# lyndonchan/wsss-analysis

Measured on AMD Instinct MI355X. Metric: images/sec CAM+CRF pseudo-labels, VOC2012 321x321, higher is better.
Workload: dtype f16x3; 1 GPU; resnet50 CAM + dense-CRF (M=21, 10 mean-field iters), 321x321, batch 32 images (=64 samples) per GPU, image-sharded; batch_images=32, num_classes=20, parallelism=image-sharded x1, no collective, steps_per_rank=239

## Files before the change

__graft_entry__.py:

```python
import os
import subprocess
import sys

ROOT = os.path.dirname(os.path.abspath(__file__))
PKG_DIR = os.path.join(ROOT, "wsss-analysis_amd")
CSRC = os.path.join(PKG_DIR, "csrc")
LIB_OUT = os.path.join(PKG_DIR, "wsscam", "libwsscam.so")
ORACLE_DIR = os.path.join(ROOT, "oracle")
ORACLE_OUT = os.path.join(ORACLE_DIR, "_build", "libdensecrf_ref.so")

HIP_SOURCES = ["api.hip", "conv_igemm.hip", "misc_kernels.hip", "net.hip", "cam_tail.hip", "crf.hip", "irn_kernels.hip", "rw.hip", "hsn.hip", "input.hip", "ir_label.hip", "stem_pool.hip", "cam_head.hip", "conv_f32.hip", "dsrg.hip", "cue_seeds.hip", "seg_eval.hip", "deeplab.hip", "seg_chain.hip", "seg_loss.hip", "pool.hip", "seg_grad.hip", "seg_sgd.hip", "seg_dropout.hip"]
EXTRA_FLAGS = {"crf.hip": ["-ffp-contract=off"], "input.hip": ["-ffp-contract=off"], "deeplab.hip": ["-ffp-contract=off"],
               "seg_chain.hip": ["-ffp-contract=off"],
               "seg_sgd.hip": ["-ffp-contract=off"],
               "seg_dropout.hip": ["-ffp-contract=off"]}


def _newer(target, deps):
    if not os.path.exists(target):
        return False
    t = os.path.getmtime(target)
    return all(os.path.getmtime(d) <= t for d in deps)


def _run(cmd):
    r = subprocess.run(cmd, stdout=subprocess.PIPE, stderr=subprocess.STDOUT, text=True)
    if r.returncode != 0:
        raise RuntimeError("command failed: %s\n%s" % (" ".join(cmd), r.stdout))
    return r.stdout


def build_lib(force=False, verbose=False):
    hipcc = os.environ.get("HIPCC", "/opt/rocm/bin/hipcc")
    objdir = os.path.join(PKG_DIR, "build")
    os.makedirs(objdir, exist_ok=True)
    os.makedirs(os.path.dirname(LIB_OUT), exist_ok=True)
    headers = [os.path.join(CSRC, "common.h"), os.path.join(CSRC, "bilerp.h"), os.path.join(CSRC, "tf_resize.h"),
               os.path.join(ROOT, "include", "wsscam.h")]
    if not force and _newer(LIB_OUT, [os.path.join(CSRC, src) for src in HIP_SOURCES] + headers):
        return LIB_OUT
    objs = []
    procs = []
    for src in HIP_SOURCES:
        sp = os.path.join(CSRC, src)
        op = os.path.join(objdir, src.replace(".hip", ".o"))
        objs.append(op)
        if not force and _newer(op, [sp] + headers):
            continue
        cmd = [hipcc, "--offload-arch=gfx950", "-O3", "-std=c++17", "-fPIC", "-Wall", "-c", sp, "-o", op] + EXTRA_FLAGS.get(src, [])
        if verbose:
            print(" ".join(cmd))
        procs.append((cmd, subprocess.Popen(cmd, stdout=subprocess.PIPE, stderr=subprocess.STDOUT, text=True)))
    for cmd, p in procs:
        out, _ = p.communicate()
        if p.returncode != 0:
            raise RuntimeError("hipcc failed: %s\n%s" % (" ".join(cmd), out))
        if verbose and out.strip():
            print(out)
    if force or procs or not _newer(LIB_OUT, objs):
        _run([hipcc, "--offload-arch=gfx950", "-shared", "-fPIC", "-o", LIB_OUT] + objs)
    return LIB_OUT


def build_oracle(force=False):
    src = os.path.join(ORACLE_DIR, "densecrf_ref.c")
    os.makedirs(os.path.dirname(ORACLE_OUT), exist_ok=True)
    if force or not _newer(ORACLE_OUT, [src]):
        _run(["gcc", "-O2", "-fPIC", "-shared", "-ffp-contract=off", "-o", ORACLE_OUT, src, "-lm"])
    return ORACLE_OUT


def build():
    build_lib()
    build_oracle()
    if PKG_DIR not in sys.path:
        sys.path.insert(0, PKG_DIR)
    import wsscam

    wsscam._lib.check_exports()


def smoke():
    if PKG_DIR not in sys.path:
        sys.path.insert(0, PKG_DIR)
    if ROOT not in sys.path:
        sys.path.insert(0, ROOT)
    from tests import smoke_impl

    smoke_impl.run()


if __name__ == "__main__":
    build_lib(force="--force" in sys.argv, verbose=True)
    build_oracle(force="--force" in sys.argv)
    print("built", LIB_OUT)
```

include/wsscam.h:

```cpp
#ifndef WSSCAM_H
#define WSSCAM_H

#include <stddef.h>
#include <stdint.h>

#ifdef __cplusplus
extern "C" {
#endif

#define WSC_VERSION 100

typedef enum wsc_status {
    WSC_OK = 0,
    WSC_ERR_INVALID = -1,
    WSC_ERR_NO_DEVICE = -2,
    WSC_ERR_HIP = -3,
    WSC_ERR_MISSING_KEY = -4,
    WSC_ERR_SHAPE = -5,
    WSC_ERR_NOMEM = -6,
    WSC_ERR_KEY_RANGE = -7,
    WSC_ERR_CAPACITY = -8,
    WSC_ERR_RANGE = -9
} wsc_status;

typedef enum wsc_arch {
    WSC_ARCH_RESNET50_CAM = 0,
    WSC_ARCH_VGG16_CAM = 1,
    WSC_ARCH_M7_CAM = 2,
    WSC_ARCH_RESNET50_IRN = 3,
    WSC_ARCH_VGG16_IRN = 4,
    WSC_ARCH_M7_IRN = 5,
    WSC_ARCH_DEEPLAB_LFOV = 6,
    WSC_ARCH_DEEPLAB_ASPP = 7
} wsc_arch;

typedef enum wsc_precision {
    WSC_PREC_BF16 = 0,
    WSC_PREC_BF16X3 = 1,
    WSC_PREC_F16 = 2,
    WSC_PREC_F16X3 = 3,
    WSC_PREC_F32 = 4
} wsc_precision;

typedef struct wsc_ctx wsc_ctx;
typedef struct wsc_net wsc_net;
typedef enum {
    WSC_OPT_CRF_GAUSS_ON_CHIP = 0,
    WSC_OPT_CRF_FUSED_BLUR = 1,
    WSC_OPT_CRF_BLUR_ON_CHIP = 2,
    WSC_OPT_CRF_RANK_BALLOT = 3,
    WSC_OPT_CRF_EMBED_FULL = 4,
    WSC_OPT_RW_TILED = 5,
    WSC_OPT_STEM_POOL_FUSED = 6,
    WSC_OPT_CONV_WINDOW = 7,
    WSC_OPT_CAM_HEAD_STREAM = 8,
    WSC_OPT_CRF_MSG_IN_UPDATE = 9,
    WSC_OPT_COUNT = 10
} wsc_option;

typedef struct wsc_crf wsc_crf;
typedef struct wsc_crf_v wsc_crf_v;

typedef struct wsc_tensor_desc {
    const char *name;
    const float *data;
    int32_t ndim;
    int64_t shape[4];
} wsc_tensor_desc;


int wsc_version(void);
const char *wsc_last_error(void);

int wsc_ctx_create(int device, void *stream, wsc_ctx **out);
void wsc_ctx_destroy(wsc_ctx *ctx);
int wsc_ctx_set_option(wsc_ctx *ctx, int option, int value);
int wsc_sync(wsc_ctx *ctx);
int wsc_ctx_range_status(wsc_ctx *ctx, int *flag_out, int clear);
int wsc_ctx_wait(wsc_ctx *ctx, wsc_ctx *other);
int wsc_ctx_mark(wsc_ctx *ctx, int slot);
int wsc_ctx_wait_mark(wsc_ctx *ctx, int slot);
int wsc_ctx_wait_for_mark(wsc_ctx *ctx, wsc_ctx *other, int slot);
int wsc_device_info(wsc_ctx *ctx, char *arch_name, size_t arch_name_len, int *num_cus);

int wsc_malloc(wsc_ctx *ctx, size_t bytes, void **dptr_out);
int wsc_free(wsc_ctx *ctx, void *dptr);
int wsc_memcpy_h2d(wsc_ctx *ctx, void *dst_dev, const void *src_host, size_t bytes);
int wsc_memcpy_d2h(wsc_ctx *ctx, void *dst_host, const void *src_dev, size_t bytes);
int wsc_memset(wsc_ctx *ctx, void *dst_dev, int value, size_t bytes);
int wsc_host_alloc(wsc_ctx *ctx, size_t bytes, void **host_out);
int wsc_host_free(wsc_ctx *ctx, void *host);
int wsc_host_write_segments(const char *path, int n, const void *const *ptrs, const size_t *sizes);
int wsc_memcpy_h2d_async(wsc_ctx *ctx, void *dst_dev, const void *src_pinned_host, size_t bytes);
int wsc_memcpy_d2h_async(wsc_ctx *ctx, void *dst_pinned_host, const void *src_dev, size_t bytes);

int wsc_timer_begin(wsc_ctx *ctx);
int wsc_timer_end(wsc_ctx *ctx, float *ms_out);

int wsc_profile_begin(wsc_ctx *ctx);
int wsc_profile_end(wsc_ctx *ctx, int max_classes, int32_t *calls_out, float *total_ms_out, double *work_out,
                    int *n_classes_out);
const char *wsc_profile_class_name(int cls);


int wsc_net_create(wsc_ctx *ctx, int arch, const wsc_tensor_desc *weights, int n_weights,
                   int num_classes, int precision, wsc_net **out);
void wsc_net_destroy(wsc_net *net);
int wsc_net_cam_size(const wsc_net *net, int S, int *h_out);
int wsc_net_feat_channels(const wsc_net *net, int *f_out);

int wsc_net_forward_cam(wsc_ctx *ctx, const wsc_net *net, const float *x_dev, int B, int S,
                        float *cam_dev, float *score_dev);
int wsc_net_cam_size_hw(const wsc_net *net, int H, int W, int *h_out, int *w_out);
int wsc_net_forward_cam_hw(wsc_ctx *ctx, const wsc_net *net, const float *x_dev, int B, int H, int W, float *cam_dev,
                           float *score_dev);

int wsc_net_forward_features(wsc_ctx *ctx, const wsc_net *net, const float *x_dev ,
                             int N, int S, float *feat_dev);

int wsc_net_forward_edge(wsc_ctx *ctx, const wsc_net *net, const float *x_dev, int B, int S, int feat_h, int feat_w,
                         float *edge_dev, float *dp_dev);

int wsc_rw_propagate(wsc_ctx *ctx, const float *x_dev, const float *edge_dev, int K, int h, int w,
                     const int32_t *dirs_host, const int32_t *path_start_host, const int32_t *path_yx_host, int D,
                     float beta, int n_steps, float *rw_dev);
int wsc_rw_propagate_batch(wsc_ctx *ctx, int n_img, const int32_t *K_host, const int32_t *h_host,
                           const int32_t *w_host, const float *x_dev, const float *edge_dev,
                           const int32_t *dirs_host, const int32_t *path_start_host, const int32_t *path_yx_host,
                           int D, float beta, int n_steps, float *rw_dev);

int wsc_net_forward_gradcam(wsc_ctx *ctx, const wsc_net *net, const float *x_dev, int N, int S, int relu,
                            float *cams_dev, float *score_dev);

#define WSC_CONV_GENERIC 0x100
int wsc_conv2d_nchw(wsc_ctx *ctx, const float *x_dev, int N, int Cin, int H, int W, const float *w_host,
                    int Cout, int kh, int kw, int stride, int pad, const float *scale_host,
                    const float *shift_host, const float *residual_dev, int relu, int precision,
                    float *y_dev);
int wsc_conv2d_nchw_dil(wsc_ctx *ctx, const float *x_dev, int N, int Cin, int H, int W, const float *w_host,
                        int Cout, int kh, int kw, int stride, int pad, int dil, const float *scale_host,
                        const float *shift_host, const float *residual_dev, int relu, int precision,
                        float *y_dev);


int wsc_net_seg_size_hw(const wsc_net *net, int H, int W, int *h_out, int *w_out);
int wsc_net_forward_seg(wsc_ctx *ctx, const wsc_net *net, const float *x_dev, int B, int H, int W, float min_prob,
                        float *fc8_dev, float *prob_dev);
int wsc_resize_bilinear_tf(wsc_ctx *ctx, const float *src_dev, int B, int h, int w, int C, float *dst_dev, int H, int W);
int wsc_pool_same_nhwc(wsc_ctx *ctx, const float *x_dev, int N, int H, int W, int C, int avg, int stride, int precision,
                       float *y_dev);
int wsc_pool_tf_nhwc(wsc_ctx *ctx, const float *x_dev, int N, int H, int W, int C, int k, int stride, int same, int precision,
                     float *y_dev);
int wsc_group_norm_nhwc(wsc_ctx *ctx, const float *x_dev, int N, int H, int W, int C, const float *gamma_host, const float *beta_host,
                        int G, float eps, int up, int relu, int Hd, int Wd, int Ctot, int coff, int precision, float *y_dev);
int wsc_maxpool_nhwc(wsc_ctx *ctx, const float *x_dev, int N, int H, int W, int C, int k, int stride, int pad, int precision,
                     float *y_dev);
int wsc_gap_linear_sigmoid(wsc_ctx *ctx, const float *feat_dev, int B, int hw, int F, const float *w_host, const float *bias_host, int C,
                           int sample_stride, int precision, float *score_dev);
int wsc_cam_flip_add(wsc_ctx *ctx, const float *head_dev, int B, int h, int w, int C, int Cs, float *cam_dev);
int wsc_irn_edge_finish(wsc_ctx *ctx, const float *e_dev, int He, int We, const float *d_dev, int Hd, int Wd, int B, int fh, int fw,
                        float ms0, float ms1, float *edge_dev, float *dp_dev);
int wsc_fc8_softmax(wsc_ctx *ctx, const float *const *fc8_dev, int n_in, long long M, int C, float min_prob, float *sum_dev,
                    float *prob_dev);

typedef struct wsc_tape_entry {
    char name[32];
    int32_t Ho, Wo, C;
    int64_t offset;
} wsc_tape_entry;
int wsc_net_seg_tape_plan(wsc_ctx *ctx, const wsc_net *net, int B, int H, int W, wsc_tape_entry *entries_out, int max_entries,
                          int *n_out, long long *tape_elems_out);
int wsc_net_forward_seg_tape(wsc_ctx *ctx, const wsc_net *net, const float *x_dev, int B, int H, int W, float min_prob,
                             float *tape_dev, long long tape_elems, float *fc8_dev, float *prob_dev);
int wsc_seg_dropout_f32(wsc_ctx *ctx, const float *x_dev, long long elems, long long first, float drop_prob, unsigned long long seed,
                        long long step, int site, float *y_dev, unsigned char *keep_dev);
int wsc_net_forward_seg_train(wsc_ctx *ctx, const wsc_net *net, const float *x_dev, int B, int H, int W, float min_prob, float drop_prob,
                              unsigned long long seed, long long step, float *tape_dev, long long tape_elems, float *fc8_dev,
                              float *prob_dev);
typedef struct wsc_seg_grad wsc_seg_grad;
typedef struct wsc_grad_entry {
    char name[32];
    int32_t kh, kw, Cin, Cout;
    int64_t w_off, b_off;
} wsc_grad_entry;
int wsc_seg_grad_create(wsc_ctx *ctx, const wsc_net *net, const wsc_tensor_desc *weights, int n_weights, wsc_seg_grad **out);
void wsc_seg_grad_destroy(wsc_seg_grad *g);
int wsc_seg_grad_layout(const wsc_seg_grad *g, wsc_grad_entry *entries_out, int max_entries, int *n_out, long long *grad_elems_out);
int wsc_net_backward_seg(wsc_ctx *ctx, wsc_seg_grad *g, int B, int H, int W, const float *tape_dev, long long tape_elems,
                         const float *dfc8_dev, float *grad_dev, long long grad_elems);
int wsc_net_backward_seg_drop(wsc_ctx *ctx, wsc_seg_grad *g, int B, int H, int W, const float *tape_dev, long long tape_elems,
                              const float *dfc8_dev, float *grad_dev, long long grad_elems, float drop_prob);
int wsc_conv2d_wgrad_nhwc(wsc_ctx *ctx, const float *x_dev, const float *dy_dev, int N, int H, int W, int Cin, int Cout, int k, int dil,
                          int splits, float *dw_dev, float *db_dev);
int wsc_conv2d_dgrad_nhwc(wsc_ctx *ctx, const float *dy_dev, const float *w_host, int N, int H, int W, int Cin, int Cout, int k, int dil,
                          float *dx_dev);
int wsc_relu_bias_grad(wsc_ctx *ctx, const float *y_dev, const float *dy_dev, long long M, int C, float *dz_dev, float *db_dev);
int wsc_relu_bias_grad_scaled(wsc_ctx *ctx, const float *y_dev, const float *dy_dev, long long M, int C, float scale, float *dz_dev,
                              float *db_dev);
int wsc_pool_same_grad_nhwc(wsc_ctx *ctx, const float *x_dev, const float *dy_dev, int N, int H, int W, int C, int avg, int stride,
                            float *dx_dev);

int wsc_seg_sgd_accumulate(wsc_ctx *ctx, wsc_seg_grad *g, const float *param_dev, const float *grad_dev, float *accum_dev,
                           long long elems, float weight_decay, int accum_num, float *l2_dev);
int wsc_seg_sgd_apply(wsc_ctx *ctx, wsc_seg_grad *g, float *param_dev, float *accum_dev, float *mom_dev, long long elems, float lr,
                      float momentum, int clear_accum);
int wsc_net_seg_load_params(wsc_ctx *ctx, wsc_net *net, wsc_seg_grad *g, const float *param_dev, long long elems);

enum { WSC_TRACE_CONV = 0, WSC_TRACE_POOL = 1, WSC_TRACE_GATHER = 2, WSC_TRACE_HEAD = 3 };
enum { WSC_TRACE_INPUT = -1 , WSC_TRACE_NONE = -2  };
typedef struct wsc_trace_op {
    int32_t kind;
    int32_t in, in2, res;
    int32_t Ho, Wo;
    int32_t C, coff, pitch;
    int32_t kh, kw, stride, pad, dil, relu;
    int32_t affine2;
    int32_t stride2;
    int32_t pool_rule, pool_k, pool_stride, pool_pad, pool_avg;
    int32_t fused_next;
    char label[100];
} wsc_trace_op;
int wsc_net_trace_plan(wsc_ctx *ctx, const wsc_net *net, int N, int H, int W, wsc_trace_op *ops_out, int max_ops, int *n_ops_out);
int wsc_net_forward_trace(wsc_ctx *ctx, const wsc_net *net, const float *x_dev, int N, int H, int W, const long long *offsets_host,
                          int n_offsets, float *trace_dev, long long trace_elems);


int wsc_cam_postprocess(wsc_ctx *ctx, const float *cam_dev, int B, int C, int h, int w,
                        const int32_t *size_hw_host , const int32_t *keys_host,
                        const int32_t *key_off_host , const int64_t *strided_off_host ,
                        const int64_t *highres_off_host , float *strided_dev, float *highres_dev);

int wsc_cam_eval_confusion(wsc_ctx *ctx, const float *highres_dev, int B, const int32_t *size_hw_host,
                           const int32_t *keys_host, const int32_t *key_off_host,
                           const int64_t *highres_off_host, float bg_thres, const uint8_t *gt_dev, int n_class,
                           int ignore_label, uint8_t *pred_dev, int64_t *confusion_dev);

int wsc_unary_from_maps(wsc_ctx *ctx, const float *maps_dev, int B, int C, int N, float bg_value,
                        float *unary_dev);

int wsc_cam_eval_confusion_nn(wsc_ctx *ctx, const float *maps_dev, int B, const int32_t *src_hw_host ,
                              const int32_t *out_hw_host , const int32_t *keys_host, const int32_t *key_off_host ,
                              const int64_t *maps_off_host , const uint8_t *gt_dev, int n_class, int ignore_label,
                              uint8_t *pred_dev, int64_t *confusion_dev);

int wsc_label_confusion_nn(wsc_ctx *ctx, const int32_t *labels_dev, int B, const int32_t *src_hw_host ,
                           const int32_t *out_hw_host , const int64_t *labels_off_host , const uint8_t *gt_dev,
                           int n_class, int ignore_label, uint8_t *pred_dev, int64_t *confusion_dev);

int wsc_sem_seg_finish(wsc_ctx *ctx, const float *rw_dev, int B, const int64_t *rw_off_host , const int32_t *khw_host ,
                       const int32_t *up_hw_host , const int32_t *out_hw_host , const int32_t *keys_host,
                       const int32_t *key_off_host , int has_bg, float bg_thres, uint8_t *label_dev);

int wsc_cam_unary(wsc_ctx *ctx, const float *cam_dev, int B, int C, int h, int w, int H0, int W0, float bg_value,
                  float *unary_dev);
int wsc_cam_unary_pm(wsc_ctx *ctx, const float *cam_dev, int B, int C, int h, int w, int H0, int W0, float bg_value,
                     float *unary_pm_dev);

int wsc_cam_sum_scales(wsc_ctx *ctx, const float *cam_dev, int n_images, int n_scales, long long map_elems, float *out_dev);

int wsc_msf_input_u8(wsc_ctx *ctx, const uint8_t *images_dev, int B, const int32_t *size_hw_host,
                     const int64_t *offset_host, int S, const float *mean3_host, const float *std3_host,
                     int pre_div255, int pair, float *x_dev);

int wsc_resize_u8(wsc_ctx *ctx, const uint8_t *images_dev, int B, const int32_t *size_hw_host, const int64_t *offset_host,
                  int OH, int OW, uint8_t *out_dev);

int wsc_bilinear_resize(wsc_ctx *ctx, const float *src_dev, int C, int h, int w, float *dst_dev, int H,
                        int W);


int wsc_label_unary_from_cam(wsc_ctx *ctx, const float *highres_dev, int B, int K, int N, float thres, float gt_prob,
                             float *unary_dev, int32_t *labels_dev);
int wsc_ir_label_combine(wsc_ctx *ctx, const int32_t *fg_pred_dev, const int32_t *bg_pred_dev, const int32_t *keys_host,
                         int B, int M, int N, uint8_t *conf_dev);


int wsc_dsrg_seed_grow(wsc_ctx *ctx, const float *tags_dev, const float *cues_dev, const float *probs_dev,
                       int B, int H, int W, int C, float th_f, float th_b, float *out_dev);

#define WSC_SEG_LOSS_SEC 0
#define WSC_SEG_LOSS_DSRG 1
enum {
    WSC_SEG_LOSS_SEED = 0,
    WSC_SEG_LOSS_CONSTRAIN,
    WSC_SEG_LOSS_EXPAND,
    WSC_SEG_LOSS_1,
    WSC_SEG_LOSS_2,
    WSC_SEG_LOSS_3,
    WSC_SEG_LOSS_NORM,
    WSC_SEG_LOSS_SEED_BG,
    WSC_SEG_LOSS_SEED_FG,
    WSC_SEG_LOSS_N
};
int wsc_seg_loss(wsc_ctx *ctx, int method , const float *prob_dev, const float *crf_dev,
                 const float *cues_dev, const float *labels_dev , int B, int H, int W, int C,
// ... 71 lines not shown
```

wsss-analysis_amd/csrc/common.h:

```cpp
#pragma once
#include <hip/hip_runtime.h>
#include <assert.h>
#include <stdint.h>
#include <map>
#include <string>
#include <unordered_map>
#include <vector>

#include "../../include/wsscam.h"

typedef uint16_t bf16_t;

typedef __bf16 bf16x8_t __attribute__((ext_vector_type(8)));
typedef _Float16 f16x8_t __attribute__((ext_vector_type(8)));
typedef float f32x16_t __attribute__((ext_vector_type(16)));
typedef float f32x4_t __attribute__((ext_vector_type(4)));

__host__ __device__ inline bf16_t f32_to_bf16(float f) {
    union { float f; uint32_t u; } v;
    v.f = f;
    uint32_t u = v.u;
    if ((u & 0x7fffffffu) > 0x7f800000u) return (bf16_t)((u >> 16) | 0x40);
    u += 0x7fffu + ((u >> 16) & 1u);
    return (bf16_t)(u >> 16);
}
__host__ __device__ inline float bf16_to_f32(bf16_t h) {
    union { float f; uint32_t u; } v;
    v.u = ((uint32_t)h) << 16;
    return v.f;
}

__host__ __device__ inline uint16_t f32_to_f16(float f) {
#if defined(__HIP_DEVICE_COMPILE__)
    const _Float16 h = (_Float16)fminf(fmaxf(f, -65504.f), 65504.f);
    return __builtin_bit_cast(uint16_t, h);
#else
    union { float f; uint32_t u; } v, magic;
    v.f = f;
    const uint32_t sign = v.u & 0x80000000u;
    v.u ^= sign;
    uint16_t o;
    if (v.u >= ((127u + 16u) << 23)) {
        o = v.u > (255u << 23) ? 0x7e00 : 0x7bff;
    } else if (v.u < (113u << 23)) {
        magic.u = ((127u - 15u) + (23u - 10u) + 1u) << 23;
        v.f += magic.f;
        o = (uint16_t)(v.u - magic.u);
    } else {
        const uint32_t mant_odd = (v.u >> 13) & 1u;
        v.u += ((15u - 127u) << 23) + 0xfffu;
        v.u += mant_odd;
        o = (uint16_t)(v.u >> 13);
        if (o >= 0x7c00) o = 0x7bff;
    }
    return (uint16_t)(o | (sign >> 16));
#endif
}
__host__ __device__ inline float f16_to_f32(uint16_t h) {
#if defined(__HIP_DEVICE_COMPILE__)
    return (float)__builtin_bit_cast(_Float16, h);
#else
    union { float f; uint32_t u; } o, magic;
    magic.u = 113u << 23;
    const uint32_t shifted_exp = 0x7c00u << 13;
    o.u = ((uint32_t)h & 0x7fffu) << 13;
    const uint32_t exp = shifted_exp & o.u;
    o.u += (127u - 15u) << 23;
    if (exp == shifted_exp) o.u += (128u - 16u) << 23;
    else if (exp == 0) { o.u += 1u << 23; o.f -= magic.f; }
    o.u |= ((uint32_t)h & 0x8000u) << 16;
    return o.f;
#endif
}
__host__ __device__ inline uint16_t f32_to_h16(float f, int fmt) { return fmt ? f32_to_f16(f) : f32_to_bf16(f); }
__host__ __device__ inline float h16_to_f32(uint16_t h, int fmt) { return fmt ? f16_to_f32(h) : bf16_to_f32(h); }

void wsc_set_error(const char *fmt, ...);
#define WSC_HIP(expr)                                                                          \
    do {                                                                                       \
        hipError_t _e = (expr);                                                                \
        if (_e != hipSuccess) {                                                                \
            wsc_set_error("%s:%d: %s failed: %s", __FILE__, __LINE__, #expr,                   \
                          hipGetErrorString(_e));                                              \
            return WSC_ERR_HIP;                                                                \
        }                                                                                      \
    } while (0)
#define WSC_CHECK(cond, code, ...)                                                             \
    do {                                                                                       \
        if (!(cond)) {                                                                         \
            wsc_set_error(__VA_ARGS__);                                                        \
            return (code);                                                                     \
        }                                                                                      \
    } while (0)
#define WSC_TRY(expr)                                                                          \
    do {                                                                                       \
        int _s = (expr);                                                                       \
        if (_s != WSC_OK) return _s;                                                           \
    } while (0)

enum WscKernelClass {
    WSC_K_CONV256 = 0,
    WSC_K_CONV128,
    WSC_K_CONV64,
    WSC_K_CONV_SMALLCIN,
    WSC_K_POOL_MISC,
    WSC_K_CAM_TAIL,
    WSC_K_CRF_BUILD,
    WSC_K_GAUSS_MSG,
    WSC_K_BLUR,
    WSC_K_SLICE_UPDATE,
    WSC_K_CRF_MISC,
    WSC_K_WGRAD,
    WSC_K_GRAD_MISC,
    WSC_K_COUNT
};
struct WscProfRecord {
    int cls;
    double work;
    hipEvent_t e0, e1;
};

struct WscGaussCache;
void wsc_gauss_cache_destroy(WscGaussCache *cache);
struct wsc_ctx {
    int device = 0;
    hipStream_t stream = nullptr;
    bool own_stream = false;
    int num_cus = 0;
    std::string arch;
    void *ws = nullptr;
    size_t ws_bytes = 0;
    static constexpr int PIN_SLOTS = 8;
    struct PinSlot {
        void *p = nullptr;
        size_t bytes = 0;
        hipEvent_t ev = nullptr;
        bool busy = false;
    };
    PinSlot pin_ring[PIN_SLOTS];
    int pin_next = 0;
    int opt[WSC_OPT_COUNT] = {1, 1, 1, 0, 0, -1, 1, 1, 1, 1};
    void *zero_page = nullptr;
    unsigned *range_host = nullptr, *range_dev = nullptr;
    hipEvent_t ev0 = nullptr, ev1 = nullptr;
    hipEvent_t join_ev = nullptr;
    hipEvent_t marks[8] = {};
    bool mark_set[8] = {};
    hipStream_t aux_stream = nullptr;
    hipEvent_t fork_ev = nullptr, aux_done_ev = nullptr;
    bool profiling = false;
    std::vector<WscProfRecord> prof;
    std::vector<hipEvent_t> prof_pool;
    std::multimap<size_t, void *> free_blocks;
    std::unordered_map<void *, size_t> live_blocks;
    WscGaussCache *gauss_cache = nullptr;
};
int wsc_ctx_workspace(wsc_ctx *ctx, size_t bytes, void **out);
int wsc_ctx_range_check(wsc_ctx *ctx);
__device__ __forceinline__ unsigned half2_at_ceiling(unsigned hw) { return (hw & 0x7fff7fffu) + 0x04010401u; }
struct WscKernelTimer {
    wsc_ctx *ctx;
    int idx = -1;
    WscKernelTimer(wsc_ctx *c, int cls, double work);
    ~WscKernelTimer();
};
int wsc_ctx_cached_alloc(wsc_ctx *ctx, size_t bytes, void **out);
void wsc_ctx_cached_free(wsc_ctx *ctx, void *p);
struct WscCachedGuard {
    wsc_ctx *ctx;
    void *p;
    WscCachedGuard(wsc_ctx *c, void *q) : ctx(c), p(q) {}
    WscCachedGuard(const WscCachedGuard &) = delete;
    WscCachedGuard &operator=(const WscCachedGuard &) = delete;
    void free_now() {
        if (p) wsc_ctx_cached_free(ctx, p);
        p = nullptr;
    }
    ~WscCachedGuard() { free_now(); }
};
int wsc_ctx_upload_small(wsc_ctx *ctx, void *dst_dev, const void *src_host, size_t bytes);
class WscStagedTable {
  public:
    explicit WscStagedTable(wsc_ctx *c) : ctx(c) {}
    WscStagedTable(const WscStagedTable &) = delete;
    WscStagedTable &operator=(const WscStagedTable &) = delete;
    ~WscStagedTable() { release(); }
    size_t add(const void *src, size_t bytes);
    template <class T> size_t add(const std::vector<T> &v) { return add(v.data(), v.size() * sizeof(T)); }
    int upload();
    template <class T> T *at(size_t off) const { return reinterpret_cast<T *>(dev + off); }
    int read_back(size_t off, void *dst, size_t bytes);
    void release() { wsc_ctx_cached_free(ctx, dev); dev = nullptr; }
  private:
    wsc_ctx *ctx;
    std::vector<char> host;
    char *dev = nullptr;
};
int wsc_set_max_dynamic_lds(wsc_ctx *ctx, const void *fn, int bytes);

constexpr int CONV_FMT_F32 = 2;
inline int conv_fmt(wsc_precision prec) {
    if (prec == WSC_PREC_F32) return CONV_FMT_F32;
    return (prec == WSC_PREC_F16 || prec == WSC_PREC_F16X3) ? 1 : 0;
}
inline size_t conv_elem_bytes(wsc_precision prec) { return prec == WSC_PREC_F32 ? sizeof(float) : sizeof(bf16_t); }
inline int conv_split(wsc_precision prec) { return prec == WSC_PREC_BF16X3 ? 1 : (prec == WSC_PREC_F16X3 ? 2 : 0); }

enum ConvForm {
    CONV_FORM_GENERIC = 0,
    CONV_FORM_SMALL2,
    CONV_FORM_SMALL4,
    CONV_FORM_STEM_ROWS
};
inline bool conv_form_dma(ConvForm f) { return f == CONV_FORM_GENERIC || f == CONV_FORM_STEM_ROWS; }

struct ConvKLayout {
    ConvForm form;
    int kh, kw;
    int kw_steps;
    int kstep;
    int ck;
    bool interleaved;
    int cchunks;
    int ksteps_base;
    int Kbase;
    int Kw;
    int nk;
    int lo_at;
    int index(int ci, int r, int s) const {
        if (form == CONV_FORM_STEM_ROWS) return r * 64 + s * 4 + ci;
        if (form == CONV_FORM_GENERIC) return (((ci / ck) * kh + r) * kw + s) * kstep + ci % ck;
        return r * (form == CONV_FORM_SMALL2 ? 4 : 8) * 4 + s * 4 + ci;
    }
};
inline ConvKLayout conv_k_layout(int kh, int kw, int Cin, ConvForm form, wsc_precision prec) {
    ConvKLayout L;
    const int split = conv_split(prec);
    L.form = form; L.kh = kh; L.kw = kw;
    L.interleaved = split == 2 && conv_form_dma(form);
    L.kstep = prec == WSC_PREC_F32 ? 32 : 64;
    L.ck = (L.interleaved || prec == WSC_PREC_F32) ? 32 : 64;
    L.kw_steps = form == CONV_FORM_STEM_ROWS ? 1 : kw;
    L.cchunks = form == CONV_FORM_GENERIC ? Cin / L.ck : 1;
    if (form == CONV_FORM_GENERIC) L.ksteps_base = kh * kw * L.cchunks;
    else if (form == CONV_FORM_STEM_ROWS) L.ksteps_base = kh;
    else L.ksteps_base = (kh * (form == CONV_FORM_SMALL2 ? 4 : 8) * 4 + L.kstep - 1) / L.kstep;
    L.Kbase = L.ksteps_base * L.kstep;
    const bool segments = split != 0 && !L.interleaved;
    L.Kw = L.Kbase * (segments ? 2 : 1);
    L.nk = L.ksteps_base * (segments ? 3 : 1);
    L.lo_at = L.interleaved ? 32 : L.Kbase;
    return L;
}
__host__ __device__ inline int conv_half_shift(float mx) {
    union { float f; uint32_t u; } v;
    v.f = mx;
    if (!(mx > 0.f) || (v.u & 0x7f800000u) == 0x7f800000u) return 0;
    const int E = (int)(v.u >> 23);
    const int e = E ? E - 126 : (31 - __builtin_clz(v.u)) - 148;
    const int sh = 13 - e;
    return sh > 100 ? 100 : (sh < -100 ? -100 : sh);
}
__host__ __device__ inline float conv_pow2(int sh) {
    union { float f; uint32_t u; } v;
    v.u = (uint32_t)(sh + 127) << 23;
    return v.f;
}
inline int conv_cout_pad(int Cout) { return Cout <= 64 ? 64 : ((Cout + 127) / 128) * 128; }
inline int conv_tile_bn(int CoutPad) { return CoutPad % 128 == 0 ? 128 : 64; }
inline void conv_stem_rows_input_dims(int Ho, int Wo, int stride, int kh, int *Hp, int *Wp) {
    *Hp = (Ho - 1) * stride + kh;
    *Wp = (Wo - 1) * stride + 8;
}

inline void conv_fastdiv(unsigned d, unsigned *mul, unsigned *s1, unsigned *s2) {
    unsigned l = 0;
    while ((1ull << l) < d) ++l;
    *mul = (unsigned)(((1ull << 32) * ((1ull << l) - d)) / d + 1);
    *s1 = l < 1 ? l : 1;
    *s2 = l > 0 ? l - 1 : 0;
}

struct Act {
    void *hi = nullptr, *lo = nullptr;
    wsc_precision prec = WSC_PREC_BF16;
    explicit operator bool() const { return hi != nullptr; }
    int fmt() const { return conv_fmt(prec); }
    int split() const { return conv_split(prec); }
    Act at(size_t elems) const {
        Act a = *this;
        a.hi = (char *)hi + elems * conv_elem_bytes(prec);
        if (lo) a.lo = (char *)lo + elems * conv_elem_bytes(prec);
        return a;
    }
    bool is_f32() const { return prec == WSC_PREC_F32; }
    bf16_t *h16() const { assert(!hi || !is_f32()); return (bf16_t *)hi; }
    bf16_t *h16_lo() const { assert(!hi || !is_f32()); return (bf16_t *)lo; }
    float *f32() const { assert(!hi || (is_f32() && !lo)); return (float *)hi; }
};
inline size_t act_bytes(size_t n, wsc_precision prec) {
    return (n * conv_elem_bytes(prec) + 255) / 256 * 256 * (conv_split(prec) ? 2 : 1);
}
inline Act act_carve(char *&cursor, size_t n, wsc_precision prec) {
    Act a;
    a.prec = prec;
    a.hi = cursor;
    if (conv_split(prec)) a.lo = cursor + act_bytes(n, prec) / 2;
    cursor += act_bytes(n, prec);
    return a;
}

struct ConvLaunch {
    Act x;
    const void *w;
    const float *s1, *b1;
    const float *s2, *b2;
    Act res;
    Act y;
    float *y_f32;
    int N, H, W, Cin, Ho, Wo, Cout, CoutPad;
    int kh, kw, stride, pad;
    int dil = 1;
    int relu;
    ConvForm form;
    wsc_precision prec;
    int generic;
    int ldy;
    Act x2;
    int H2, W2, C2, stride2;
    bool operands_match() const {
        for (const Act *a : {&x, &res, &y, &x2})
            if (*a && a->prec != prec) return false;
        return true;
    }
};
int conv_igemm_launch(wsc_ctx *ctx, const ConvLaunch &p);
int conv_f32_launch(wsc_ctx *ctx, const ConvLaunch &p);
int launch_cam_head(wsc_ctx *ctx, Act x, int M, int K, const bf16_t *w, int Kw, int CoutPad, const float *s1, const float *b1,
                    int C, int relu, float *y);

inline int wsc_grid_for(long long total, int block = 256, int cap = 256 * 16) {
    long long g = (total + block - 1) / block;
    if (g > cap) g = cap;
    if (g < 1) g = 1;
    return (int)g;
}
int launch_nchw_to_nhwc4(wsc_ctx *ctx, const float *x, int N, int H, int W, Act y);
void stem_pool_input_dims(int H, int W, int *Hp, int *Wp);
int launch_stem_pool(wsc_ctx *ctx, Act x, int N, int H, int W, const bf16_t *w, int Kw, const float *s1, const float *b1, int relu,
                     Act y);
int launch_gather_strided(wsc_ctx *ctx, Act x, int N, int H, int W, int C, int stride, int Ho, int Wo, Act y, int ldy);
int launch_nchw_to_nhwc4_pad(wsc_ctx *ctx, const float *x, int N, int H, int W, int Hp, int Wp, int pad, Act y);
int launch_flip_add(wsc_ctx *ctx, const float *head, int B, int h, int w, int C, int Cs, float *cam);
int launch_gap_linear_sigmoid(wsc_ctx *ctx, Act feat, int B, int hw, int F, const float *Wc, const float *bias, int C, float *score,
                              int sample_stride);
int launch_act_to_f32(wsc_ctx *ctx, Act x, size_t n, float *y);
int launch_nchw_to_nhwc(wsc_ctx *ctx, const float *x, int N, int C, int HW, Act y);
int launch_nhwc_to_nchw(wsc_ctx *ctx, Act x, int N, int C, int HW, float *y);

enum PoolRule { POOL_TORCH, POOL_TF_SAME, POOL_TF_VALID };
struct PoolGeom {
    int k, stride, pad_t, pad_l, Ho, Wo;
    bool avg;
};
inline bool pool_axis(PoolRule rule, int in, int k, int stride, int pad, int *out, int *pad_before) {
    *out = *pad_before = 0;
    if (in < 1 || k < 1 || stride < 1) return false;
    if (rule == POOL_TF_SAME) {
        *out = (in + stride - 1) / stride;
        const int pad_total = (*out - 1) * stride + k - in;
        *pad_before = pad_total > 0 ? pad_total / 2 : 0;
    } else if (rule == POOL_TF_VALID) {
        *out = in >= k ? (in - k) / stride + 1 : 0;
    } else {
        if (pad < 0) return false;
        *pad_before = pad;
        *out = (in + 2 * pad - k) / stride + 1;
    }
    return *out >= 1;
}
inline bool pool_geom(PoolRule rule, int k, int stride, int pad , bool avg, int H, int W, PoolGeom *g) {
    g->k = k; g->stride = stride; g->avg = avg;
    const bool okh = pool_axis(rule, H, k, stride, pad, &g->Ho, &g->pad_t), okw = pool_axis(rule, W, k, stride, pad, &g->Wo, &g->pad_l);
    return okh && okw;
}
int launch_pool(wsc_ctx *ctx, Act x, int N, int H, int W, int C, const PoolGeom &g, Act y);

int launch_pool_grad(wsc_ctx *ctx, const float *x, const float *dy, int N, int H, int W, int C, const PoolGeom &g, float *dx);

struct WgradPlan {
    int M, nk, pad;
    bool small_cin;
    int bn, tiles_ci, tiles_co;
    int ntaps;
    unsigned long long taps;
    unsigned dead;
    int splits;
    long long out_elems, slab_elems;
};
int wgrad_plan(const wsc_ctx *ctx, int N, int H, int W, int Cin, int Cout, int k, int dil, int splits, WgradPlan *pl);
int wgrad_launch(wsc_ctx *ctx, const WgradPlan &pl, const float *x, const float *dz, int H, int W, int Cin, int Cout, int k, int dil,
                 float *slab, float *dw);
int relu_bias_grad_blocks(long long M);
int launch_relu_bias_grad(wsc_ctx *ctx, const float *y, const float *dy, long long M, int C, float scale, float *dz, float *partial,
                          float *db);
int launch_copy_channels(wsc_ctx *ctx, const float *src, long long M, int Cs, int Cd, float *dst);
inline int dgrad_cz(int Cout) { return (Cout + 31) / 32 * 32; }
void dgrad_pack(const float *w_hwio, int k, int Cin, int Cout, std::vector<float> *packed);
int dgrad_launch(wsc_ctx *ctx, const float *dz, const float *w_packed, const float *ones, const float *zeros, int N, int H, int W, int Cin,
                 int Cout, int k, int dil, const float *sum_with, float *dx);

struct SgdSegment {
    long long start;
    float mult;
    int decay;
};
constexpr int SGD_MAX_SEGMENTS = 128;
constexpr int SGD_L2_MAX_BLOCKS = 1024;
int sgd_accumulate_launch(wsc_ctx *ctx, const SgdSegment *segs_dev, int n_segs, const float *param, const float *grad, float *accum,
                          long long elems, float weight_decay, int accum_num, double *l2_partials, unsigned *l2_counter, float *l2_dev);
int sgd_apply_launch(wsc_ctx *ctx, float *param, float *accum, float *mom, long long elems, float lr, float momentum, int clear_accum);
struct RepackJob {
    long long w_off, b_off;
    int k, Cin, Cout;
    int small;
    int kstep, Kw, lo_at, nsteps;
    int rot_Kw;
    int splits, rows_per;
    int max_block0, pack_block0, rot_block0;
    int tiles;
    long long pmax_off;
    void *wp;
    float *s1, *b1, *w_rot;
};
struct RepackPlan {
    RepackJob *jobs_dev = nullptr;
    int n_jobs = 0, small_job = -1, small_tiles = 0;
    int ck = 0;
    int max_blocks = 0, pack_blocks = 0, rot_blocks = 0;
    long long pmax_elems = 0;
    float *pmax = nullptr;
    wsc_precision prec = WSC_PREC_BF16;
    double bytes = 0;
};
int repack_plan(std::vector<RepackJob> &jobs, wsc_precision prec, RepackPlan *plan);
int repack_launch(wsc_ctx *ctx, const RepackPlan &plan, const float *param);

int seg_dropout_check(const char *fn, float drop_prob, long long step);
float seg_dropout_scale(float drop_prob);
int launch_seg_dropout_f32(wsc_ctx *ctx, const float *x, float *y, float *tape, uint8_t *keep, long long n, unsigned long long first,
                           float drop_prob, unsigned long long seed, unsigned step, unsigned site);
int launch_seg_dropout(wsc_ctx *ctx, Act a, size_t n, int Cout, float drop_prob, unsigned long long seed, unsigned step, unsigned site,
                       float *tape);

int launch_nhwc3_to_nhwc4(wsc_ctx *ctx, const float *x, int N, int H, int W, Act y);
int launch_fc8_softmax(wsc_ctx *ctx, const float *const *in, int n_in, long long M, int C, float min_prob, float *fc8, float *prob);

constexpr int SEG_MAX_C = 32;

int launch_group_norm_stats(wsc_ctx *ctx, const float *x, int N, int H, int W, int C, int G, float eps, void *partial,
                            void *stats);
size_t group_norm_partial_bytes(int N, int H, int W, int G);
int launch_group_norm_apply(wsc_ctx *ctx, const float *x, const void *stats, const float *gamma, const float *beta,
                            int N, int H, int W, int C, int G, int up, int relu, Act y, int Hd, int Wd, int Ctot, int coff);
int launch_edge_finish(wsc_ctx *ctx, const float *e, int He, int We, const float *d, int Hd, int Wd, int B, int fh, int fw,
                       float ms0, float ms1, float *edge, float *dp);
```

wsss-analysis_amd/csrc/conv_igemm.hip:

```cpp
#include "common.h"

#include <type_traits>

namespace {

constexpr int BK = 64;

struct ConvKArgs {
    const bf16_t *x, *x_lo, *w;
    const float *s1, *b1, *s2, *b2;
    const bf16_t *res, *res_lo;
    bf16_t *y, *y_lo;
    float *y_f32;
    int H, W, Cin, Ho, Wo, Cout;
    int ldy;
    int kh, kw, stride, pad, relu;
    int M, HoWo;
    int m_base, m_end;
    unsigned div_howo_mul, div_howo_s1, div_howo_s2, div_wo_mul, div_wo_s1, div_wo_s2;
    int cchunks;
    int dil;
    int ksteps_base;
    int nk;
    int Kw;
    int Kbase;
    int ntiles_n, nblocks;
    const bf16_t *zero;
    int spare1;
    long long lo_delta;
    const bf16_t *x2;
    long long lo_delta2;
    int cc2, H2, W2, C2, stride2;
    int ldx;
    int win_npix;
    int spare2, spare3;
    unsigned *range;
};

__device__ __forceinline__ int lds_off(int row, int slot) {
    return row * 128 + ((slot ^ ((row >> 1) & 7)) << 4);
}

__device__ __forceinline__ void decode_row(const ConvKArgs &p, int m, int &n, int &ho, int &wo) {
    const unsigned t1 = __umulhi(p.div_howo_mul, (unsigned)m);
    n = (int)((t1 + (((unsigned)m - t1) >> p.div_howo_s1)) >> p.div_howo_s2);
    const int rem = m - n * p.HoWo;
    const unsigned t2 = __umulhi(p.div_wo_mul, (unsigned)rem);
    ho = (int)((t2 + (((unsigned)rem - t2) >> p.div_wo_s1)) >> p.div_wo_s2);
    wo = rem - ho * p.Wo;
}

template <int BM, int BN, int MODE, int SPLIT, int ET, int STAGES, int FAST = 0, int WPT = 0>
__global__ __launch_bounds__(BM * 2, (STAGES == 1 && FAST != 0) ? 4 : 2) void conv_igemm_kernel(ConvKArgs p) {
    constexpr bool GLDS = MODE == 0;
    constexpr int WMT = BM == 256 ? 128 : 64;
    constexpr bool FEPI = (FAST & 1) != 0, PW = (FAST & 2) != 0;
    constexpr bool WIN = WPT > 0;
    static_assert(!WIN || (SPLIT == 2 && BM == 128 && STAGES == 2 && FAST == 1), "LDS window: single-staged split, 128-row tile");
    static_assert(FAST == 0 || (SPLIT != 1 && ET == 1 && (MODE == 0 || FAST == 1)),
                  "FAST paths: f16, one plane or the single-staged split; the pointwise prologue belongs to the LDS-DMA layers");
    static_assert(SPLIT != 2 || (MODE == 0 && STAGES == 2), "single-staged split: LDS-DMA layers, two LDS buffers");
    static_assert(STAGES == 2 || SPLIT == 0, "one LDS buffer serves a one-K-step layer, which a layer of three K segments never is");
    constexpr int CK = SPLIT == 2 ? 32 : 64;
    constexpr int NT = BM * 2;
    constexpr int NW = BM / 32;
    constexpr int WR = BM / WMT;
    constexpr int WC = NW / WR;
    constexpr int WN = BN / WC;
    constexpr int MI = WMT / 32;
    constexpr int NI = WN / 32;
    static_assert(WR * WC == NW && WN % 32 == 0, "wave layout");
    constexpr int NB = BN * 8 / NT;
    constexpr int A_BYTES = BM * BK * 2;
    constexpr int B_BYTES = BN * BK * 2;
    constexpr int WIN_BYTES = WPT * 4096;
    constexpr int A_REGION = WIN ? WIN_BYTES : STAGES * A_BYTES;
    constexpr int CT_STRIDE = BN + 4;
    static_assert(GLDS || (BM == 128 && STAGES <= 2), "register staging exists for the 128-row tile only");
    static_assert(STAGES >= 1 && STAGES <= 2, "1 (single K-step layers) or 2 LDS buffers");

    extern __shared__ __attribute__((aligned(16))) char smem[];

    const int t = threadIdx.x;
    const int lane = t & 63;
    const int wv = __builtin_amdgcn_readfirstlane(t >> 6);
    const int wm = wv / WC, wn = wv - wm * WC;

    int tile;
    {
        const int bid = blockIdx.x;
        const int xcd = bid & 7;
        const int q = p.nblocks >> 3, r = p.nblocks & 7;
        tile = (xcd < r ? xcd * (q + 1) : r * (q + 1) + (xcd - r) * q) + (bid >> 3);
    }
    const int mt = tile / p.ntiles_n;
    const int nt = tile - mt * p.ntiles_n;
    const int m0 = p.m_base + mt * BM;
    const int n0 = nt * BN;

    const int slot = t & 7;
    const int lrow = GLDS ? (wv * 32 + (lane >> 3)) : (t >> 3);
    constexpr int RSTEP = GLDS ? 8 : 32;
    int hb[4], wb[4];
    long long base[4];
#pragma unroll
    for (int i = 0; i < 4; ++i) {
        const int m = m0 + lrow + RSTEP * i;
        if (PW) {
            const int mc = m < p.m_end ? m : p.m_end - 1;
            hb[i] = 0;
            wb[i] = 0;
            base[i] = (long long)mc * p.ldx;
        } else if (m < p.m_end) {
            int n, ho, wo;
            decode_row(p, m, n, ho, wo);
            hb[i] = ho * p.stride - p.pad;
            wb[i] = wo * p.stride - p.pad;
            base[i] = (((long long)n * p.H + hb[i]) * p.W + wb[i]) * (long long)p.ldx;
        } else {
            hb[i] = -(1 << 28);
            wb[i] = 0;
            base[i] = 0;
        }
    }
    const int brow0 = GLDS ? (wv * (BN / NW) + (lane >> 3)) : (t >> 3);
    const bf16_t *wrow[NB];
#pragma unroll
    for (int i = 0; i < NB; ++i) {
        const int r = brow0 + RSTEP * i;
        const int ks = GLDS ? (slot ^ ((r >> 1) & 7)) : slot;
        wrow[i] = p.w + (long long)(n0 + r) * p.Kw + ks * 8;
    }

    long long aoff[4];
#pragma unroll
    for (int i = 0; i < 4; ++i) {
        const int r = lrow + RSTEP * i;
        const int ks = slot ^ ((r >> 1) & 7);
        if (SPLIT == 2) aoff[i] = base[i] + (ks & 3) * 8 + ((ks & 4) ? p.lo_delta : 0ll);
        else aoff[i] = base[i] + ks * 8;
    }

    typedef unsigned u32x4_t __attribute__((ext_vector_type(4)));
    u32x4_t ra[4], rb[NB];

    auto load_tile = [&](int kt) __attribute__((always_inline)) {
        int seg = 0, ktl = kt;
        if (SPLIT) {
            seg = kt / p.ksteps_base;
            ktl = kt - seg * p.ksteps_base;
        }
        const bf16_t *src = (SPLIT && seg == 1) ? p.x_lo : p.x;
        const int g = ktl * 8 + slot;
        const int khi = g >> MODE;
        const int px = (g & ((1 << MODE) - 1)) * 2;
#pragma unroll
        for (int i = 0; i < 4; ++i) {
            const int hi = hb[i] + khi, wi = wb[i] + px;
            const bool okh = khi < p.kh && (unsigned)hi < (unsigned)p.H;
            const uint2 *q = reinterpret_cast<const uint2 *>(src + base[i] + ((long long)khi * p.W + px) * 4);
            uint2 v0 = make_uint2(0, 0), v1 = make_uint2(0, 0);
            if (okh && (unsigned)wi < (unsigned)p.W) v0 = q[0];
            if (okh && (unsigned)(wi + 1) < (unsigned)p.W) v1 = q[1];
            ra[i] = u32x4_t{v0.x, v0.y, v1.x, v1.y};
        }
        const int wk = ((SPLIT && seg == 2) ? p.Kbase : 0) + ktl * 64;
#pragma unroll
        for (int i = 0; i < NB; ++i) rb[i] = *reinterpret_cast<const u32x4_t *>(wrow[i] + wk);
    };

    auto store_lds = [&](int buf) __attribute__((always_inline)) {
        char *sa = smem + buf * A_BYTES;
        char *sb = smem + STAGES * A_BYTES + buf * B_BYTES;
#pragma unroll
        for (int i = 0; i < 4; ++i) *reinterpret_cast<u32x4_t *>(sa + lds_off(lrow + 32 * i, slot)) = ra[i];
#pragma unroll
        for (int i = 0; i < NB; ++i) *reinterpret_cast<u32x4_t *>(sb + lds_off(lrow + 32 * i, slot)) = rb[i];
    };

    f32x16_t acc[MI][NI];
#pragma unroll
    for (int mi = 0; mi < MI; ++mi)
#pragma unroll
        for (int ni = 0; ni < NI; ++ni)
#pragma unroll
            for (int r = 0; r < 16; ++r) acc[mi][ni][r] = 0.f;

    const int l31 = lane & 31;
    const int kgrp = lane >> 5;

    auto mfma = [&](const u32x4_t &a, const u32x4_t &b, f32x16_t &c) {
        if (ET == 0)
            c = __builtin_amdgcn_mfma_f32_32x32x16_bf16(__builtin_bit_cast(bf16x8_t, a), __builtin_bit_cast(bf16x8_t, b),
                                                        c, 0, 0, 0);
// ... 777 lines not shown
```

wsss-analysis_amd/csrc/net.hip:

```cpp
#include "common.h"

#include <algorithm>
#include <cmath>
#include <cstring>
#include <unordered_map>

namespace {

struct HostTensor {
    const float *data;
    int ndim;
    int64_t shape[4];
    int64_t numel() const {
        int64_t n = 1;
        for (int i = 0; i < ndim; ++i) n *= shape[i];
        return n;
    }
};
typedef std::unordered_map<std::string, HostTensor> Dict;

struct ConvW {
    void *w = nullptr;
    float *s1 = nullptr, *b1 = nullptr, *s2 = nullptr, *b2 = nullptr;
    int Cin = 0, Cout = 0, CoutPad = 0, kh = 1, kw = 1, stride = 1, pad = 0, relu = 0;
// ... 95 lines not shown
        HostTensor t;
        t.data = weights[i].data;
        t.ndim = weights[i].ndim;
        for (int k = 0; k < 4; ++k) t.shape[k] = k < t.ndim ? weights[i].shape[k] : 1;
        if (t.ndim == 0) { t.ndim = 1; t.shape[0] = 1; }
        (*d)[weights[i].name] = t;
    }
    return WSC_OK;
}

int fold_bn(const Dict &d, const std::string &bn, int C, double eps_default, std::vector<float> &s,
            std::vector<float> &b) {
    const HostTensor *g, *be, *mu, *var;
    WSC_TRY(get(d, bn + ".weight", 1, &g));
    WSC_TRY(get(d, bn + ".bias", 1, &be));
    WSC_TRY(get(d, bn + ".running_mean", 1, &mu));
    WSC_TRY(get(d, bn + ".running_var", 1, &var));
    WSC_CHECK(g->shape[0] == C && be->shape[0] == C && mu->shape[0] == C && var->shape[0] == C, WSC_ERR_SHAPE,
              "state_dict: batch-norm '%s' is not %d channels", bn.c_str(), C);
    double eps = eps_default;
    auto it = d.find(bn + ".eps");
    if (it != d.end() && it->second.data) eps = it->second.data[0];
    s.resize(C);
    b.resize(C);
    for (int c = 0; c < C; ++c) {
        const double sc = (double)g->data[c] / std::sqrt((double)var->data[c] + eps);
        s[c] = (float)sc;
        b[c] = (float)((double)be->data[c] - (double)mu->data[c] * sc);
    }
    return WSC_OK;
}

int make_conv(wsc_net *net, const HostTensor *w, int stride, int pad, int relu, ConvForm form,
              const std::vector<float> &s1, const std::vector<float> &b1, const std::vector<float> *s2,
              const std::vector<float> *b2, ConvW *out) {
    const int Cout = (int)w->shape[0], Cin = (int)w->shape[1], kh = (int)w->shape[2], kw = (int)w->shape[3];
    ConvW c;
    c.Cout = Cout;
    c.CoutPad = conv_cout_pad(Cout);
    c.kh = kh; c.kw = kw; c.stride = stride; c.pad = pad; c.relu = relu; c.form = form;
    if (form == CONV_FORM_GENERIC) {
        WSC_CHECK(Cin % 64 == 0, WSC_ERR_SHAPE, "conv with Cin=%d is not supported (need a multiple of 64)", Cin);
        c.Cin = Cin;
    } else if (form == CONV_FORM_STEM_ROWS) {
        WSC_CHECK(Cin <= 4 && kw <= 7 && conv_split(net->prec) == 2, WSC_ERR_SHAPE, "padded-stem conv needs Cin <= 4, kw <= 7, f16x3");
        c.Cin = 4;
    } else {
        WSC_CHECK(Cin <= 4, WSC_ERR_SHAPE, "small-Cin conv needs Cin <= 4, got %d", Cin);
        WSC_CHECK(kw <= (form == CONV_FORM_SMALL2 ? 4 : 8), WSC_ERR_SHAPE, "small-Cin conv: kw=%d too wide", kw);
        c.Cin = 4;
    }
    const ConvKLayout lay = conv_k_layout(kh, kw, c.Cin, form, net->prec);
    const int Kw = lay.Kw;
    const bool f32 = net->prec == WSC_PREC_F32;
    const int fmt = conv_fmt(net->prec), split = conv_split(net->prec);
    std::vector<char> wp((size_t)c.CoutPad * Kw * conv_elem_bytes(net->prec), 0);
    std::vector<float> s1v(s1);
    std::vector<float> wscale(Cout, 1.f);
    if (fmt == 1) {
        const size_t per = (size_t)Cin * kh * kw;
        for (int co = 0; co < Cout; ++co) {
            float mx = 0.f;
            for (size_t i = 0; i < per; ++i) mx = std::max(mx, std::fabs(w->data[(size_t)co * per + i]));
            const int sh = conv_half_shift(mx);
            wscale[co] = conv_pow2(sh);
            s1v[co] = s1[co] * conv_pow2(-sh);
        }
    }
    for (int co = 0; co < Cout; ++co) {
        bf16_t *row = f32 ? nullptr : (bf16_t *)wp.data() + (size_t)co * Kw;
        float *row_f32 = f32 ? (float *)wp.data() + (size_t)co * Kw : nullptr;
        const float wsc = wscale[co];
        auto put = [&](int k, float v) {
            if (f32) {
                row_f32[k] = v;
                return;
            }
            v *= wsc;
            const bf16_t h = f32_to_h16(v, fmt);
            row[k] = h;
            if (split) row[lay.lo_at + k] = f32_to_h16(v - h16_to_f32(h, fmt), fmt);
        };
        for (int ci = 0; ci < Cin; ++ci)
            for (int r = 0; r < kh; ++r)
                for (int s = 0; s < kw; ++s) put(lay.index(ci, r, s), w->data[(((size_t)co * Cin + ci) * kh + r) * kw + s]);
    }
    WSC_TRY(upload(net, wp.data(), wp.size(), &c.w));
    auto up_vec = [&](const std::vector<float> &v, float **dst) -> int {
        std::vector<float> p(c.CoutPad, 0.f);
        for (int i = 0; i < Cout; ++i) p[i] = v[i];
        return upload(net, p.data(), p.size() * sizeof(float), (void **)dst);
    };
    WSC_TRY(up_vec(s1v, &c.s1));
    WSC_TRY(up_vec(b1, &c.b1));
    if (s2) {
        WSC_TRY(up_vec(*s2, &c.s2));
        WSC_TRY(up_vec(*b2, &c.b2));
    }
    *out = c;
    return WSC_OK;
}

ConvLaunch conv_launch(const ConvW &c, wsc_precision prec) {
    ConvLaunch L = {};
    L.w = c.w; L.s1 = c.s1; L.b1 = c.b1; L.s2 = c.s2; L.b2 = c.b2;
    L.Cin = c.Cin; L.Cout = c.Cout; L.CoutPad = c.CoutPad;
    L.kh = c.kh; L.kw = c.kw; L.stride = c.stride; L.pad = c.pad; L.relu = c.relu; L.dil = c.dil;
    L.form = c.form; L.prec = prec;
    return L;
}
void on_padded_input(ConvLaunch &L, int in_h, int in_w) {
    L.H = in_h; L.W = in_w; L.pad = 0;
}

int add_conv_op(wsc_net *net, const std::string &label, const ConvW &c, int in, int out, int res, int in2 = -1, int stride2 = 0) {
    net->convs.push_back(c);
    Op op;
    op.label = label;
    op.type = OP_CONV; op.conv = (int)net->convs.size() - 1; op.in = in; op.out = out; op.res = res; op.in2 = in2; op.ps = stride2;
    net->ops.push_back(op);
    return WSC_OK;
}
void add_pool_op(wsc_net *net, PoolRule rule, int k, int stride, int pad, bool avg, int in, int out) {
    Op op;
    int n_pools = 0;
    for (const Op &o : net->ops) n_pools += o.type == OP_POOL;
    op.label = "pool:" + std::to_string(n_pools);
    op.type = OP_POOL; op.in = in; op.out = out; op.rule = rule; op.pk = k; op.ps = stride; op.pp = pad; op.avg = avg;
    net->ops.push_back(op);
}
void add_gather_op(wsc_net *net, const std::string &label, int stride, int in, int out, int pitch, int coff) {
    Op op;
    op.label = label;
    op.type = OP_GATHER; op.in = in; op.out = out; op.ps = stride; op.pitch = pitch; op.coff = coff;
    net->ops.push_back(op);
}

int resnet_conv(wsc_net *net, const Dict &d, const std::string &conv, const std::string &bn, int stride, int pad,
                int relu, ConvForm form, int in, int out, int res) {
    const HostTensor *w;
    WSC_TRY(get(d, conv + ".weight", 4, &w));
    std::vector<float> s, b;
    WSC_TRY(fold_bn(d, bn, (int)w->shape[0], 1e-5, s, b));
    ConvW c;
    WSC_TRY(make_conv(net, w, stride, pad, relu, form, s, b, nullptr, nullptr, &c));
    return add_conv_op(net, conv, c, in, out, res);
}

int build_resnet50_backbone(wsc_net *net, const Dict &d) {
    WSC_TRY(resnet_conv(net, d, "resnet50.conv1", "resnet50.bn1", 2, 3, 1, conv_split(net->prec) == 2 ? CONV_FORM_STEM_ROWS : CONV_FORM_SMALL4, -1, 0, -1));
    add_pool_op(net, POOL_TORCH, 3, 2, 1, false, 0, 1);
    net->taps.push_back((int)net->ops.size() - 1);
    int cur = 1;
    const int blocks[4] = {3, 4, 6, 3};
    const int strides[4] = {1, 2, 2, 1};
    for (int L = 0; L < 4; ++L) {
        for (int bi = 0; bi < blocks[L]; ++bi) {
            const std::string pre = "resnet50.layer" + std::to_string(L + 1) + "." + std::to_string(bi);
            const int s = bi == 0 ? strides[L] : 1;
            int f[3], nf = 0;
            for (int i = 0; i < 4 && nf < 3; ++i)
                if (i != cur) f[nf++] = i;
            WSC_TRY(resnet_conv(net, d, pre + ".conv1", pre + ".bn1", 1, 0, 1, CONV_FORM_GENERIC, cur, f[0], -1));
            bool fuse_here = false;
            if (net->prec != WSC_PREC_F32 && has(d, pre + ".downsample.0.weight") && has(d, pre + ".conv3.weight")) {
                const HostTensor *w3, *wd;
                WSC_TRY(get(d, pre + ".conv3.weight", 4, &w3));
                WSC_TRY(get(d, pre + ".downsample.0.weight", 4, &wd));
                fuse_here = wd->shape[0] == w3->shape[0] && w3->shape[2] == 1 && w3->shape[3] == 1 && wd->shape[2] == 1 &&
                            wd->shape[3] == 1 && w3->shape[1] % 8 == 0 && wd->shape[1] % 8 == 0 &&
                            (w3->shape[1] + wd->shape[1]) % 64 == 0;
            }
            if (fuse_here) {
                const HostTensor *w3, *wd;
                WSC_TRY(get(d, pre + ".conv3.weight", 4, &w3));
                WSC_TRY(get(d, pre + ".downsample.0.weight", 4, &wd));
                const int Co = (int)w3->shape[0], K1 = (int)w3->shape[1], K2 = (int)wd->shape[1];
                std::vector<float> s3, b3, sd, bd;
                WSC_TRY(fold_bn(d, pre + ".bn3", Co, 1e-5, s3, b3));
                WSC_TRY(fold_bn(d, pre + ".downsample.1", Co, 1e-5, sd, bd));
                std::vector<float> wc((size_t)Co * (K1 + K2)), sig(Co), sh(Co);
                for (int co = 0; co < Co; ++co) {
                    float g = std::max(std::fabs(s3[co]), std::fabs(sd[co]));
                    if (!(g > 0.f)) g = 1.f;
                    sig[co] = g;
                    sh[co] = b3[co] + bd[co];
                    for (int k = 0; k < K1; ++k) wc[(size_t)co * (K1 + K2) + k] = w3->data[(size_t)co * K1 + k] * (s3[co] / g);
                    for (int k = 0; k < K2; ++k) wc[(size_t)co * (K1 + K2) + K1 + k] = wd->data[(size_t)co * K2 + k] * (sd[co] / g);
                }
                HostTensor wt;
                wt.data = wc.data(); wt.ndim = 4; wt.shape[0] = Co; wt.shape[1] = K1 + K2; wt.shape[2] = 1; wt.shape[3] = 1;
                WSC_TRY(resnet_conv(net, d, pre + ".conv2", pre + ".bn2", s, 1, 1, CONV_FORM_GENERIC, f[0], f[1], -1));
                ConvW c;
                WSC_TRY(make_conv(net, &wt, 1, 0, 1, CONV_FORM_GENERIC, sig, sh, nullptr, nullptr, &c));
                if (conv_split(net->prec) != 1) {
                    WSC_TRY(add_conv_op(net, pre + ".conv3+downsample", c, f[1], f[0], -1, cur, s));
                } else {
                    net->ops.back().pitch = K1 + K2;
                    net->ops.back().coff = 0;
                    add_gather_op(net, pre + ".gather", s, cur, f[1], K1 + K2, K1);
                    WSC_TRY(add_conv_op(net, pre + ".conv3+downsample", c, f[1], f[0], -1));
                }
                cur = f[0];
                continue;
            }
            WSC_TRY(resnet_conv(net, d, pre + ".conv2", pre + ".bn2", s, 1, 1, CONV_FORM_GENERIC, f[0], f[1], -1));
            int res = cur;
            if (has(d, pre + ".downsample.0.weight")) {
                WSC_TRY(resnet_conv(net, d, pre + ".downsample.0", pre + ".downsample.1", s, 0, 0, CONV_FORM_GENERIC, cur, f[2], -1));
                res = f[2];
            }
            WSC_TRY(resnet_conv(net, d, pre + ".conv3", pre + ".bn3", 1, 0, 1, CONV_FORM_GENERIC, f[1], f[0], res));
            cur = f[0];
        }
        net->taps.push_back((int)net->ops.size() - 1);
    }
    net->final_buf = cur;
    return WSC_OK;
}

int build_resnet50(wsc_net *net, const Dict &d) {
    WSC_TRY(build_resnet50_backbone(net, d));
    const HostTensor *cw;
    WSC_TRY(get(d, "classifier.weight", 4, &cw));
    WSC_CHECK(cw->shape[0] == net->C && cw->shape[2] == 1 && cw->shape[3] == 1, WSC_ERR_SHAPE,
              "classifier.weight must be [%d][F][1][1]", net->C);
    net->F = (int)cw->shape[1];
    std::vector<float> one(net->C, 1.f), zero(net->C, 0.f);
    WSC_TRY(make_conv(net, cw, 1, 0, 0, CONV_FORM_GENERIC, one, zero, nullptr, nullptr, &net->head));
    return WSC_OK;
}

int read_pool_spec(const Dict &d, int n_pools, std::vector<PoolSpec> *spec, bool *present) {
    *present = has(d, "pool_spec");
    if (!*present) return WSC_OK;
    const HostTensor *t;
    WSC_TRY(get(d, "pool_spec", 2, &t));
    WSC_CHECK(t->shape[0] == n_pools && t->shape[1] == 3, WSC_ERR_SHAPE, "pool_spec must be [%d][3] (window, stride, same) for this arch, got [%lld][%lld]",
              n_pools, (long long)t->shape[0], (long long)t->shape[1]);
    for (int i = 0; i < n_pools; ++i) {
        const float *r = t->data + 3 * i;
        WSC_CHECK(r[0] == std::floor(r[0]) && r[1] == std::floor(r[1]) && r[2] == std::floor(r[2]), WSC_ERR_INVALID,
                  "pool_spec row %d: (%g, %g, %g) is not integral", i, (double)r[0], (double)r[1], (double)r[2]);
        const PoolSpec ps = {(int)r[0], (int)r[1], (int)r[2]};
        WSC_CHECK((ps.k == 2 || ps.k == 3) && (ps.stride == 1 || ps.stride == 2) && ps.stride <= ps.k && (ps.same == 0 || ps.same == 1),
                  WSC_ERR_INVALID, "pool_spec row %d: window %d (2 / 3), stride %d (1 / 2, <= window), same %d (0 / 1)", i, ps.k, ps.stride, ps.same);
        spec->push_back(ps);
    }
    return WSC_OK;
}

int build_plain_stack(wsc_net *net, const Dict &d, const std::string &root,
                      const std::vector<std::pair<std::string, std::vector<int>>> &cfg, int *cur_io,
                      int *feat_channels, std::vector<int> *layer_taps = nullptr, const std::vector<PoolSpec> *pools = nullptr) {
    int cur = *cur_io;
    int in_ch = 3;
    bool first = true;
    size_t n_pool = 0;
    for (const auto &layer : cfg) {
        int idx = 0;
        for (int v : layer.second) {
            if (v == -1) {
                const int out = (cur + 1) & 1;
                if (pools) {
                    WSC_CHECK(n_pool < pools->size(), WSC_ERR_INVALID, "internal: pool_spec has %d rows, the stack more pools", (int)pools->size());
                    const PoolSpec &ps = (*pools)[n_pool++];
                    add_pool_op(net, ps.rule(), ps.k, ps.stride, 0, false, cur, out);
                } else add_pool_op(net, POOL_TORCH, 2, 2, 0, false, cur, out);
                cur = out;
                idx += 1;
            } else if (v == -2) {
                idx += 1;
            } else {
                const std::string key = root + "." + layer.first + "." + std::to_string(idx);
                const HostTensor *w, *bias;
                WSC_TRY(get(d, key + ".weight", 4, &w));
                WSC_TRY(get(d, key + ".bias", 1, &bias));
                WSC_CHECK(w->shape[0] == v && w->shape[1] == in_ch && w->shape[2] == 3 && w->shape[3] == 3,
                          WSC_ERR_SHAPE, "'%s.weight' must be [%d][%d][3][3]", key.c_str(), v, in_ch);
                std::vector<float> one(v, 1.f), bb(bias->data, bias->data + v);
                const std::string bn = root + "." + layer.first + "." + std::to_string(idx + 2);
                ConvW c;
                if (has(d, bn + ".running_mean")) {
                    std::vector<float> s2, b2;
                    WSC_TRY(fold_bn(d, bn, v, 1e-3, s2, b2));
                    WSC_TRY(make_conv(net, w, 1, 1, 1, first ? CONV_FORM_SMALL2 : CONV_FORM_GENERIC, one, bb, &s2, &b2, &c));
                    idx += 3;
                } else {
                    WSC_TRY(make_conv(net, w, 1, 1, 1, first ? CONV_FORM_SMALL2 : CONV_FORM_GENERIC, one, bb, nullptr, nullptr, &c));
                    idx += 2;
                }
                const int in = first ? -1 : cur;
                const int out = first ? 0 : ((cur + 1) & 1);
                WSC_TRY(add_conv_op(net, key, c, in, out, -1));
                cur = out;
                in_ch = v;
                first = false;
            }
        }
        if (layer_taps) layer_taps->push_back((int)net->ops.size() - 1);
    }
    *cur_io = cur;
    *feat_channels = in_ch;
    return WSC_OK;
}

int gradcam_bias(const Dict &d, int C, std::vector<float> &bias) {
    bias.assign(C, 0.f);
    if (!has(d, "gradcam_bias")) return WSC_OK;
    const HostTensor *gb;
    WSC_TRY(get(d, "gradcam_bias", 1, &gb));
    WSC_CHECK(gb->shape[0] == C, WSC_ERR_SHAPE, "gradcam_bias must be [%d]", C);
    for (int c = 0; c < C; ++c) bias[c] = gb->data[c];
    return WSC_OK;
}
// ... 200 lines not shown
    out->dil = dil;
    return WSC_OK;
}

int build_deeplab(wsc_net *net, const Dict &d, bool aspp) {
    struct Item { const char *name; int v; };
    const Item trunk[] = {{"conv1_1", 1}, {"conv1_2", 1}, {"", 2}, {"conv2_1", 1}, {"conv2_2", 1}, {"", 2},
                          {"conv3_1", 1}, {"conv3_2", 1}, {"conv3_3", 1}, {"", 2}, {"conv4_1", 1}, {"conv4_2", 1}, {"conv4_3", 1}, {"", 1},
                          {"conv5_1", 2}, {"conv5_2", 2}, {"conv5_3", 2}, {"", 1}, {"", 0}};
    int cur = 0, in_ch = 3;
    bool first = true;
    for (const Item &it : trunk) {
        if (it.name[0] == 0) {
            const int out = (cur + 1) & 1;
            add_pool_op(net, POOL_TF_SAME, 3, it.v == 0 ? 1 : it.v, 0, it.v == 0, cur, out);
            cur = out;
            continue;
        }
        ConvW c;
        WSC_TRY(deeplab_conv(net, d, it.name, 3, in_ch, 0, it.v, 1, first ? CONV_FORM_SMALL2 : CONV_FORM_GENERIC, &c));
        const int out = first ? 0 : ((cur + 1) & 1);
        WSC_TRY(add_conv_op(net, it.name, c, first ? -1 : cur, out, -1));
        cur = out;
        in_ch = c.Cout;
        first = false;
    }
    net->final_buf = cur;
    net->F = in_ch;
    const int rates_aspp[4] = {6, 12, 18, 24};
    const int nb = aspp ? 4 : 1;
    for (int k = 0; k < nb; ++k) {
        const std::string sfx = aspp ? "_" + std::to_string(k + 1) : "";
        SegBranch br;
        WSC_TRY(deeplab_conv(net, d, "fc6" + sfx, 3, in_ch, 0, aspp ? rates_aspp[k] : 12, 1, CONV_FORM_GENERIC, &br.fc6));
        WSC_TRY(deeplab_conv(net, d, "fc7" + sfx, 1, br.fc6.Cout, 0, 1, 1, CONV_FORM_GENERIC, &br.fc7));
        WSC_TRY(deeplab_conv(net, d, "fc8" + sfx, 1, br.fc7.Cout, net->C, 1, 0, CONV_FORM_GENERIC, &br.fc8));
        net->seg.push_back(br);
    }
    return WSC_OK;
}

inline size_t align_up(size_t v, size_t a) { return (v + a - 1) / a * a; }

struct OpDims {
    int H, W, C;
    int Ho, Wo, Co;
    int H2, W2, C2;
};
struct Plan {
    std::vector<OpDims> ops;
    size_t max_act = 0;
    int hf = 0, wf = 0;
    size_t out_elems(int N, int op) const { return (size_t)N * ops[op].Ho * ops[op].Wo * ops[op].Co; }
};

int plan_dims(const wsc_net *net, int N, int SH, int SW, Plan *pl);
int plan_dims(const wsc_net *net, int N, int S, Plan *pl) { return plan_dims(net, N, S, S, pl); }
int plan_dims(const wsc_net *net, int N, int SH, int SW, Plan *pl) {
    int bh[4] = {0, 0, 0, 0}, bw[4] = {0, 0, 0, 0}, bc[4] = {0, 0, 0, 0};
    pl->max_act = 0;
    for (const Op &op : net->ops) {
        OpDims d = {};
        d.H = op.in < 0 ? SH : bh[op.in]; d.W = op.in < 0 ? SW : bw[op.in]; d.C = op.in < 0 ? 4 : bc[op.in];
        if (op.type == OP_CONV) {
            const ConvW &c = net->convs[op.conv];
            d.Ho = (d.H + 2 * c.pad - ((c.kh - 1) * c.dil + 1)) / c.stride + 1;
            d.Wo = (d.W + 2 * c.pad - ((c.kw - 1) * c.dil + 1)) / c.stride + 1;
            d.Co = op.pitch ? op.pitch : c.Cout;
            if (op.in2 >= 0) {
                d.H2 = bh[op.in2]; d.W2 = bw[op.in2]; d.C2 = bc[op.in2];
                WSC_CHECK(c.kh == 1 && c.kw == 1 && c.stride == 1 && (d.H - 1) * op.ps < d.H2 && (d.W - 1) * op.ps < d.W2,
                          WSC_ERR_INVALID, "internal: second input of a %d x %d layer does not cover its %d x %d output", c.kh, c.kw, d.H, d.W);
            }
            WSC_CHECK(d.C + d.C2 == c.Cin, WSC_ERR_INVALID, "internal: channel mismatch %d vs %d", d.C + d.C2, c.Cin);
        } else if (op.type == OP_GATHER) {
            d.Ho = (d.H - 1) / op.ps + 1;
            d.Wo = (d.W - 1) / op.ps + 1;
            d.Co = op.pitch;
            WSC_CHECK(d.Ho == bh[op.out] && d.Wo == bw[op.out] && bc[op.out] == op.pitch && op.coff + d.C <= op.pitch, WSC_ERR_INVALID,
                      "internal: gather into a %d x %d x %d tensor does not fit", bh[op.out], bw[op.out], bc[op.out]);
        } else {
            PoolGeom g;
            pool_geom(op.rule, op.pk, op.ps, op.pp, op.avg, d.H, d.W, &g);
            d.Ho = g.Ho; d.Wo = g.Wo; d.Co = d.C;
        }
        WSC_CHECK(d.Ho > 0 && d.Wo > 0, WSC_ERR_INVALID, "input size %d x %d too small for this network", SH, SW);
        bh[op.out] = d.Ho; bw[op.out] = d.Wo; bc[op.out] = d.Co;
        pl->ops.push_back(d);
        pl->max_act = std::max(pl->max_act, pl->out_elems(N, (int)pl->ops.size() - 1));
    }
    pl->hf = bh[net->final_buf];
    pl->wf = bw[net->final_buf];
    return WSC_OK;
}

size_t taps_bytes(const wsc_net *net, const Plan &pl, int N) {
    size_t b = 0;
    for (int op : net->taps) b += act_bytes(pl.out_elems(N, op), net->prec);
    return b;
}

bool stem_pool_fused(const wsc_ctx *ctx, const wsc_net *net) {
    if (net->ops.empty() || net->ops[0].type != OP_CONV || net->ops[0].in >= 0 || net->convs[net->ops[0].conv].form != CONV_FORM_STEM_ROWS)
        return false;
    const ConvW &c0 = net->convs[net->ops[0].conv];
    bool tapped = false;
    for (int tp : net->taps) tapped = tapped || tp == 0;
    return ctx->opt[WSC_OPT_STEM_POOL_FUSED] && net->ops.size() > 1 && net->ops[1].type == OP_POOL &&
           net->ops[1].in == net->ops[0].out && net->ops[1].rule == POOL_TORCH && !net->ops[1].avg && net->ops[1].pk == 3 &&
           net->ops[1].ps == 2 && net->ops[1].pp == 1 &&
           c0.kh == 7 && c0.kw == 7 && c0.stride == 2 && c0.pad == 3 && c0.Cout == 64 && c0.s2 == nullptr &&
           net->ops[0].res < 0 && conv_fmt(net->prec) == 1 && !tapped;
}

struct TraceSink {
    const long long *off;
    float *out;
};

int run_backbone(wsc_ctx *ctx, const wsc_net *net, const float *x_dev, int N, int S, size_t extra_bytes, Act *feat, int *hf, int *wf,
                 void **extra, std::vector<Act> *taps = nullptr, int SW = 0, bool nhwc_in = false, Act *spare = nullptr,
                 const TraceSink *trace = nullptr, Act *xin_out = nullptr) {
    if (SW <= 0) SW = S;
    Plan pl;
    WSC_TRY(plan_dims(net, N, S, SW, &pl));
    int in_h = S, in_w = SW, in_pad = 0;
    bool fused_stem = false;
    if (!net->ops.empty() && net->ops[0].type == OP_CONV && net->ops[0].in < 0 && net->convs[net->ops[0].conv].form == CONV_FORM_STEM_ROWS) {
        const ConvW &c0 = net->convs[net->ops[0].conv];
        conv_stem_rows_input_dims(pl.ops[0].Ho, pl.ops[0].Wo, c0.stride, c0.kh, &in_h, &in_w);
        in_pad = c0.pad;
        fused_stem = stem_pool_fused(ctx, net);
        if (fused_stem) {
            stem_pool_input_dims(S, SW, &in_h, &in_w);
            in_pad = 5;
        }
    }
    const size_t in_elems = (size_t)N * in_h * in_w * 4;
    void *ws;
    WSC_TRY(wsc_ctx_workspace(ctx, act_bytes(in_elems, net->prec) + 4 * act_bytes(pl.max_act, net->prec) + align_up(extra_bytes, 256), &ws));
    char *p = (char *)ws;
    const Act xin = act_carve(p, in_elems, net->prec);
    Act buf[4];
    for (Act &b : buf) b = act_carve(p, pl.max_act, net->prec);
    if (taps)
        for (int op : net->taps) taps->push_back(act_carve(p, pl.out_elems(N, op), net->prec));
    *extra = (void *)p;

    if (nhwc_in) {
        WSC_CHECK(in_pad == 0, WSC_ERR_INVALID, "internal: an NHWC input has no padded-stem form");
        WSC_TRY(launch_nhwc3_to_nhwc4(ctx, x_dev, N, S, SW, xin));
    } else if (in_pad > 0) WSC_TRY(launch_nchw_to_nhwc4_pad(ctx, x_dev, N, S, SW, in_h, in_w, in_pad, xin));
    else WSC_TRY(launch_nchw_to_nhwc4(ctx, x_dev, N, S, SW, xin));
    for (size_t i = 0; i < net->ops.size(); ++i) {
        const Op &op = net->ops[i];
        const OpDims &d = pl.ops[i];
        const Act src = op.in < 0 ? xin : buf[op.in];
        if (fused_stem && i == 0) continue;
        if (fused_stem && i == 1) {
            const ConvW &c0 = net->convs[net->ops[0].conv];
            WSC_TRY(launch_stem_pool(ctx, xin, N, S, SW, (const bf16_t *)c0.w, conv_k_layout(c0.kh, c0.kw, c0.Cin, c0.form, net->prec).Kw, c0.s1,
                                     c0.b1, c0.relu, buf[op.out]));
        } else if (op.type == OP_CONV) {
            const ConvW &c = net->convs[op.conv];
            ConvLaunch L = conv_launch(c, net->prec);
            L.x = src;
            if (op.res >= 0) L.res = buf[op.res];
            L.y = buf[op.out].at(op.coff);
            L.ldy = op.pitch;
            if (op.in2 >= 0) {
                L.x2 = buf[op.in2];
                L.H2 = d.H2; L.W2 = d.W2; L.C2 = d.C2; L.stride2 = op.ps;
            }
            L.N = N; L.H = d.H; L.W = d.W; L.Ho = d.Ho; L.Wo = d.Wo;
            if (c.form == CONV_FORM_STEM_ROWS && op.in < 0) on_padded_input(L, in_h, in_w);
            WSC_TRY(conv_igemm_launch(ctx, L));
        } else if (op.type == OP_GATHER) {
            WSC_TRY(launch_gather_strided(ctx, src, N, d.H, d.W, d.C, op.ps, d.Ho, d.Wo, buf[op.out].at(op.coff), op.pitch));
        } else {
            PoolGeom g;
            WSC_CHECK(pool_geom(op.rule, op.pk, op.ps, op.pp, op.avg, d.H, d.W, &g), WSC_ERR_INVALID, "internal: a pool plan_dims let through");
            WSC_TRY(launch_pool(ctx, src, N, d.H, d.W, d.C, g, buf[op.out]));
        }
        if (trace && trace->off[i] >= 0) WSC_TRY(launch_act_to_f32(ctx, buf[op.out], pl.out_elems(N, (int)i), trace->out + trace->off[i]));
        if (taps)
            for (size_t k = 0; k < net->taps.size(); ++k)
                if (net->taps[k] == (int)i) {
                    const size_t nb = pl.out_elems(N, (int)i) * conv_elem_bytes(net->prec);
                    WSC_HIP(hipMemcpyAsync((*taps)[k].hi, buf[op.out].hi, nb, hipMemcpyDeviceToDevice, ctx->stream));
                    if (buf[op.out].lo) WSC_HIP(hipMemcpyAsync((*taps)[k].lo, buf[op.out].lo, nb, hipMemcpyDeviceToDevice, ctx->stream));
                }
    }
    *feat = buf[net->final_buf];
    if (xin_out) *xin_out = xin;
    if (spare) *spare = buf[net->final_buf == 3 ? 2 : 3];
    *hf = pl.hf;
    *wf = pl.wf;
    return WSC_OK;
}

int run_classifier(wsc_ctx *ctx, const wsc_net *net, Act feat, Act spare, int N, int count, int sample_stride, int hf, int wf,
                   float *score_dev) {
    int hw = hf * wf;
    if (net->cls_max && net->cls_pool_set) {
        const PoolSpec &ps = net->cls_pool;
        PoolGeom g;
        WSC_CHECK(pool_geom(ps.rule(), ps.k, ps.stride, 0, false, hf, wf, &g), WSC_ERR_INVALID,
                  "the %d x %d feature map is smaller than the classifier branch's %d x %d VALID pool", hf, wf, ps.k, ps.k);
        const bool crops = !ps.same && ((g.Ho - 1) * ps.stride + ps.k < hf || (g.Wo - 1) * ps.stride + ps.k < wf);
        if (crops) {
            WSC_TRY(launch_pool(ctx, feat, N, hf, wf, net->F, g, spare));
            feat = spare;
            hw = g.Ho * g.Wo;
        }
    }
    return launch_gap_linear_sigmoid(ctx, feat, count, net->cls_max ? -hw : hw, net->F, net->cls_w, net->cls_b, net->Ccls, score_dev,
                                     sample_stride);
}

}

extern "C" {

int wsc_net_create(wsc_ctx *ctx, int arch, const wsc_tensor_desc *weights, int n_weights, int num_classes,
                   int precision, wsc_net **out) {
    WSC_CHECK(ctx && weights && out && n_weights > 0, WSC_ERR_INVALID, "wsc_net_create: null argument");
    WSC_CHECK(num_classes > 0 && num_classes <= 64, WSC_ERR_INVALID, "num_classes=%d outside [1,64]", num_classes);
    wsc_precision prec;
    WSC_TRY(decode_precision(precision, &prec));
    WSC_HIP(hipSetDevice(ctx->device));
    Dict d;
    WSC_TRY(descs_to_dict(weights, n_weights, &d));
    WSC_CHECK(!has(d, "pool_spec") || arch == WSC_ARCH_VGG16_CAM || arch == WSC_ARCH_M7_CAM, WSC_ERR_INVALID,
              "pool_spec is a key of WSC_ARCH_VGG16_CAM / WSC_ARCH_M7_CAM only (arch %d)", arch);
    wsc_net *net = new wsc_net();
    net->ctx = ctx;
    net->arch = arch;
    net->C = num_classes;
    net->prec = prec;
    int st;
    switch (arch) {
    case WSC_ARCH_RESNET50_CAM: st = build_resnet50(net, d); break;
    case WSC_ARCH_VGG16_CAM: st = build_vgg16(net, d); break;
    case WSC_ARCH_M7_CAM: st = build_m7(net, d); break;
    case WSC_ARCH_RESNET50_IRN: st = build_resnet50_irn(net, d); break;
    case WSC_ARCH_VGG16_IRN: st = build_vgg16_irn(net, d); break;
    case WSC_ARCH_M7_IRN: st = build_m7_irn(net, d); break;
    case WSC_ARCH_DEEPLAB_LFOV: st = build_deeplab(net, d, false); break;
    case WSC_ARCH_DEEPLAB_ASPP: st = build_deeplab(net, d, true); break;
    default:
        wsc_set_error("unknown arch %d", arch);
        st = WSC_ERR_INVALID;
    }
    if (st != WSC_OK) {
        wsc_net_destroy(net);
        return st;
    }
    *out = net;
    return WSC_OK;
}

void wsc_net_destroy(wsc_net *net) {
    if (!net) return;
    for (void *p : net->allocs) (void)hipFree(p);
    delete net;
}

int wsc_net_cam_size(const wsc_net *net, int S, int *h_out) {
    WSC_CHECK(net && h_out, WSC_ERR_INVALID, "wsc_net_cam_size: null argument");
    Plan pl;
    WSC_TRY(plan_dims(net, 1, S, &pl));
    *h_out = pl.hf;
    return WSC_OK;
}

int wsc_net_feat_channels(const wsc_net *net, int *f_out) {
    WSC_CHECK(net && f_out, WSC_ERR_INVALID, "wsc_net_feat_channels: null argument");
    *f_out = net->F;
    return WSC_OK;
}

int wsc_net_cam_size_hw(const wsc_net *net, int H, int W, int *h_out, int *w_out) {
    WSC_CHECK(net && h_out && w_out, WSC_ERR_INVALID, "wsc_net_cam_size_hw: null argument");
    Plan pl;
    WSC_TRY(plan_dims(net, 1, H, W, &pl));
    *h_out = pl.hf;
    *w_out = pl.wf;
    return WSC_OK;
}

static int run_head(wsc_ctx *ctx, const ConvLaunch &L) {
    if (conv_fmt(L.prec) == 1 && L.Cout <= 32 && L.CoutPad >= 32 && L.Cin % 256 == 0 && L.y_f32 != nullptr &&
        ctx->opt[WSC_OPT_CAM_HEAD_STREAM] != 0) {
        WSC_CHECK(L.operands_match(), WSC_ERR_INVALID, "cam head: the input is not of the layer's precision %d", (int)L.prec);
        const int st = launch_cam_head(ctx, L.x, L.N * L.Ho * L.Wo, L.Cin, (const bf16_t *)L.w,
                                       conv_k_layout(L.kh, L.kw, L.Cin, L.form, L.prec).Kw, L.CoutPad, L.s1, L.b1, L.Cout, L.relu, L.y_f32);
        if (st != WSC_ERR_INVALID) return st;
    }
    return conv_igemm_launch(ctx, L);
}

int wsc_net_forward_cam(wsc_ctx *ctx, const wsc_net *net, const float *x_dev, int B, int S, float *cam_dev,
                        float *score_dev) {
    return wsc_net_forward_cam_hw(ctx, net, x_dev, B, S, S, cam_dev, score_dev);
}

int wsc_net_forward_cam_hw(wsc_ctx *ctx, const wsc_net *net, const float *x_dev, int B, int S, int SW, float *cam_dev,
                           float *score_dev) {
    WSC_CHECK(ctx && net && x_dev && cam_dev, WSC_ERR_INVALID, "wsc_net_forward_cam: null argument");
    WSC_CHECK(B > 0 && S > 0 && SW > 0, WSC_ERR_INVALID, "wsc_net_forward_cam: B=%d input %d x %d", B, S, SW);
    WSC_CHECK(net->head.w != nullptr, WSC_ERR_INVALID, "wsc_net_forward_cam: the network has no CAM head (a segmentation net: wsc_net_forward_seg)");
    WSC_CHECK(score_dev == nullptr || net->cls_w != nullptr, WSC_ERR_INVALID,
              "this architecture has no classifier branch (score_dev must be NULL)");
    WSC_HIP(hipSetDevice(ctx->device));
    const int N = 2 * B;
    Plan pl;
    WSC_TRY(plan_dims(net, N, S, SW, &pl));
    const size_t head_bytes = (size_t)N * pl.hf * pl.wf * net->C * sizeof(float);
    Act feat, spare;
    int hf, wf;
    void *extra;
    WSC_TRY(run_backbone(ctx, net, x_dev, N, S, head_bytes, &feat, &hf, &wf, &extra, nullptr, SW, false, &spare));
    float *head_out = (float *)extra;
    ConvLaunch L = conv_launch(net->head, net->prec);
    L.x = feat;
    L.y_f32 = head_out;
    L.N = N; L.H = hf; L.W = wf; L.Ho = hf; L.Wo = wf;
    WSC_TRY(run_head(ctx, L));
    WSC_TRY(launch_flip_add(ctx, head_out, B, hf, wf, net->C, net->C, cam_dev));
// ... 635 lines not shown
                              const float *dfc8_dev, float *grad_dev, long long grad_elems, float drop_prob) {
    WSC_TRY(seg_dropout_check("wsc_net_backward_seg_drop", drop_prob, 0));
    return backward_seg("wsc_net_backward_seg_drop", ctx, g, B, H, W, tape_dev, tape_elems, dfc8_dev, grad_dev, grad_elems,
                        seg_dropout_scale(drop_prob));
}

namespace {
int sgd_check(const char *fn, const wsc_ctx *ctx, const wsc_seg_grad *g, long long elems, bool pointers) {
    WSC_CHECK(ctx && g && pointers, WSC_ERR_INVALID, "%s: null argument", fn);
    WSC_CHECK(ctx == g->ctx, WSC_ERR_INVALID, "%s: the context is not the one the wsc_seg_grad was created on", fn);
    WSC_CHECK(elems == g->grad_elems, WSC_ERR_INVALID, "%s: buffers of %lld floats, the layout has %lld", fn, elems, g->grad_elems);
    return WSC_OK;
}
}

int wsc_seg_sgd_accumulate(wsc_ctx *ctx, wsc_seg_grad *g, const float *param_dev, const float *grad_dev, float *accum_dev, long long elems,
                           float weight_decay, int accum_num, float *l2_dev) {
    WSC_TRY(sgd_check("wsc_seg_sgd_accumulate", ctx, g, elems, param_dev && grad_dev && accum_dev));
    WSC_CHECK(accum_num >= 1, WSC_ERR_INVALID, "wsc_seg_sgd_accumulate: accum_num=%d", accum_num);
    WSC_HIP(hipSetDevice(ctx->device));
    return sgd_accumulate_launch(ctx, g->segs, g->n_segs, param_dev, grad_dev, accum_dev, elems, weight_decay, accum_num, g->l2_partials,
                                 g->l2_counter, l2_dev);
}

int wsc_seg_sgd_apply(wsc_ctx *ctx, wsc_seg_grad *g, float *param_dev, float *accum_dev, float *mom_dev, long long elems, float lr,
                      float momentum, int clear_accum) {
    WSC_TRY(sgd_check("wsc_seg_sgd_apply", ctx, g, elems, param_dev && accum_dev && mom_dev));
    WSC_HIP(hipSetDevice(ctx->device));
    return sgd_apply_launch(ctx, param_dev, accum_dev, mom_dev, elems, lr, momentum, clear_accum);
}

int wsc_net_seg_load_params(wsc_ctx *ctx, wsc_net *net, wsc_seg_grad *g, const float *param_dev, long long elems) {
    WSC_CHECK(ctx && net && g && param_dev, WSC_ERR_INVALID, "wsc_net_seg_load_params: null argument");
    WSC_CHECK(!net->seg.empty(), WSC_ERR_INVALID, "wsc_net_seg_load_params: the network is not a WSC_ARCH_DEEPLAB_* net");
    WSC_CHECK(g->net == net, WSC_ERR_INVALID, "wsc_net_seg_load_params: the wsc_seg_grad was created for another net");
    WSC_TRY(sgd_check("wsc_net_seg_load_params", ctx, g, elems, true));
    std::vector<ConvW *> convs;
    for (const Op &op : net->ops)
        if (op.type == OP_CONV) convs.push_back(&net->convs[op.conv]);
    for (SegBranch &br : net->seg) {
        convs.push_back(&br.fc6);
        convs.push_back(&br.fc7);
        convs.push_back(&br.fc8);
    }
    WSC_CHECK(convs.size() == g->layers.size(), WSC_ERR_INVALID, "internal: %d layers of the net, %d of the layout", (int)convs.size(),
              (int)g->layers.size());
    for (size_t i = 0; i < convs.size(); ++i) {
        const ConvW &c = *convs[i];
        const GradLayer &L = g->layers[i];
        WSC_CHECK(c.kh == L.k && c.kw == L.k && c.Cout == L.Cout && (c.form == CONV_FORM_GENERIC ? c.Cin == L.Cin : (c.Cin == 4 && L.Cin <= 4)) &&
                      !c.s2 && !c.b2,
                  WSC_ERR_INVALID, "internal: layer '%s' of the layout is not the net's", L.name.c_str());
    }
    WSC_HIP(hipSetDevice(ctx->device));
    if (!g->repack.jobs_dev) {
        std::vector<RepackJob> jobs(convs.size());
        for (size_t i = 0; i < convs.size(); ++i) {
            const ConvW &c = *convs[i];
            const GradLayer &L = g->layers[i];
            RepackJob &J = jobs[i];
            J = RepackJob();
            J.w_off = L.w_off; J.b_off = L.b_off;
            J.k = L.k; J.Cin = L.Cin; J.Cout = L.Cout;
            J.small = c.form != CONV_FORM_GENERIC;
            J.wp = c.w; J.s1 = c.s1; J.b1 = c.b1;
            J.w_rot = L.w_rot;
        }
        RepackPlan plan;
        WSC_TRY(repack_plan(jobs, net->prec, &plan));
        void *jd = nullptr, *pm = nullptr;
        WSC_HIP(hipMalloc(&jd, jobs.size() * sizeof(RepackJob)));
        g->allocs.push_back(jd);
        WSC_HIP(hipMemcpy(jd, jobs.data(), jobs.size() * sizeof(RepackJob), hipMemcpyHostToDevice));
        if (plan.pmax_elems > 0) {
            WSC_HIP(hipMalloc(&pm, (size_t)plan.pmax_elems * sizeof(float)));
            g->allocs.push_back(pm);
        }
        plan.pmax = (float *)pm;
        plan.jobs_dev = (RepackJob *)jd;
        g->repack = plan;
    }
    return repack_launch(ctx, g->repack, param_dev);
}

int wsc_conv2d_nchw(wsc_ctx *ctx, const float *x_dev, int N, int Cin, int H, int W, const float *w_host, int Cout,
                    int kh, int kw, int stride, int pad, const float *scale_host, const float *shift_host,
                    const float *residual_dev, int relu, int precision, float *y_dev) {
    return wsc_conv2d_nchw_dil(ctx, x_dev, N, Cin, H, W, w_host, Cout, kh, kw, stride, pad, 1, scale_host, shift_host, residual_dev, relu,
                               precision, y_dev);
}

int wsc_conv2d_nchw_dil(wsc_ctx *ctx, const float *x_dev, int N, int Cin, int H, int W, const float *w_host, int Cout, int kh, int kw,
                        int stride, int pad, int dil, const float *scale_host, const float *shift_host, const float *residual_dev,
                        int relu, int precision, float *y_dev) {
    WSC_CHECK(ctx && x_dev && w_host && y_dev, WSC_ERR_INVALID, "wsc_conv2d_nchw: null argument");
    WSC_CHECK(dil >= 1 && (dil == 1 || (Cin > 4 && stride >= 1)), WSC_ERR_INVALID,
              "wsc_conv2d_nchw: dilation %d (>= 1; > 1 on the generic form only, Cin a multiple of 64)", dil);
    WSC_CHECK(Cout % 8 == 0, WSC_ERR_INVALID, "wsc_conv2d_nchw: Cout=%d must be a multiple of 8", Cout);
    WSC_HIP(hipSetDevice(ctx->device));
    wsc_net tmp;
    tmp.ctx = ctx;
    const int generic = (precision & WSC_CONV_GENERIC) ? 1 : 0;
    wsc_precision prec;
    WSC_TRY(decode_precision(precision & ~WSC_CONV_GENERIC, &prec));
    tmp.prec = prec;
    HostTensor wt;
    wt.data = w_host; wt.ndim = 4; wt.shape[0] = Cout; wt.shape[1] = Cin; wt.shape[2] = kh; wt.shape[3] = kw;
    std::vector<float> s1(Cout, 1.f), b1(Cout, 0.f);
    if (scale_host) s1.assign(scale_host, scale_host + Cout);
    if (shift_host) b1.assign(shift_host, shift_host + Cout);
    ConvForm form = CONV_FORM_GENERIC;
    if (Cin <= 4) form = kw <= 4 ? CONV_FORM_SMALL2 : CONV_FORM_SMALL4;
    if (form == CONV_FORM_SMALL4 && conv_split(prec) == 2 && (stride & 1) == 0 && kw <= 7) form = CONV_FORM_STEM_ROWS;
    ConvW c;
    int st = make_conv(&tmp, &wt, stride, pad, relu, form, s1, b1, nullptr, nullptr, &c);
    auto cleanup = [&]() {
        (void)hipStreamSynchronize(ctx->stream);
        for (void *p : tmp.allocs) (void)hipFree(p);
    };
    if (st != WSC_OK) { cleanup(); return st; }
    c.dil = dil;
    const int Ho = (H + 2 * pad - ((kh - 1) * dil + 1)) / stride + 1, Wo = (W + 2 * pad - ((kw - 1) * dil + 1)) / stride + 1;
    if (Ho < 1 || Wo < 1) {
        cleanup();
        wsc_set_error("wsc_conv2d_nchw: a %d x %d input is too small for this kernel, padding and dilation", H, W);
        return WSC_ERR_INVALID;
    }
    int in_h = H, in_w = W;
    if (form == CONV_FORM_STEM_ROWS) conv_stem_rows_input_dims(Ho, Wo, stride, kh, &in_h, &in_w);
    const size_t in_e = (size_t)N * in_h * in_w * c.Cin, out_e = (size_t)N * Ho * Wo * Cout;
    void *ws;
    st = wsc_ctx_workspace(ctx, act_bytes(in_e, prec) + 2 * act_bytes(out_e, prec), &ws);
    if (st != WSC_OK) { cleanup(); return st; }
    char *p = (char *)ws;
    const Act xi = act_carve(p, in_e, prec), yo = act_carve(p, out_e, prec);
    const Act ri = residual_dev ? act_carve(p, out_e, prec) : Act();
    if (form == CONV_FORM_STEM_ROWS) st = launch_nchw_to_nhwc4_pad(ctx, x_dev, N, H, W, in_h, in_w, pad, xi);
    else if (form != CONV_FORM_GENERIC) st = launch_nchw_to_nhwc4(ctx, x_dev, N, H, W, xi);
    else st = launch_nchw_to_nhwc(ctx, x_dev, N, Cin, H * W, xi);
    if (st == WSC_OK && residual_dev) st = launch_nchw_to_nhwc(ctx, residual_dev, N, Cout, Ho * Wo, ri);
    if (st == WSC_OK) {
        ConvLaunch L = conv_launch(c, prec);
        L.x = xi; L.res = ri; L.y = yo;
        L.N = N; L.H = H; L.W = W; L.Ho = Ho; L.Wo = Wo;
        if (form == CONV_FORM_STEM_ROWS) on_padded_input(L, in_h, in_w);
        L.generic = generic;
        st = conv_igemm_launch(ctx, L);
    }
    if (st == WSC_OK) st = launch_nhwc_to_nchw(ctx, yo, N, Cout, Ho * Wo, y_dev);
    cleanup();
    return st;
}

int wsc_group_norm_nhwc(wsc_ctx *ctx, const float *x_dev, int N, int H, int W, int C, const float *gamma_host, const float *beta_host,
                        int G, float eps, int up, int relu, int Hd, int Wd, int Ctot, int coff, int precision, float *y_dev) {
    WSC_CHECK(ctx && x_dev && gamma_host && beta_host && y_dev, WSC_ERR_INVALID, "wsc_group_norm_nhwc: null argument");
    wsc_precision prec;
    WSC_TRY(decode_precision(precision, &prec));
    WSC_CHECK(N > 0 && H > 0 && W > 0 && C > 0 && G > 0 && C % G == 0, WSC_ERR_INVALID,
              "wsc_group_norm_nhwc: %d x %d x %d x %d in %d groups", N, H, W, C, G);
    WSC_CHECK(up == 1 || up == 2 || up == 4, WSC_ERR_INVALID, "wsc_group_norm_nhwc: upsample factor %d (1, 2 or 4)", up);
    WSC_CHECK(Hd >= 1 && Wd >= 1 && Hd <= H * up && Wd <= W * up, WSC_ERR_INVALID,
              "wsc_group_norm_nhwc: crop %d x %d of a %d x %d map", Hd, Wd, H * up, W * up);
    WSC_CHECK(coff >= 0 && Ctot >= 1 && coff <= Ctot - C, WSC_ERR_INVALID, "wsc_group_norm_nhwc: channels [%d, %d + %d) of %d", coff, coff, C,
              Ctot);
    WSC_CHECK(prec != WSC_PREC_F32 || (C % 4 == 0 && Ctot % 4 == 0 && coff % 4 == 0 && ((uintptr_t)x_dev & 15) == 0), WSC_ERR_INVALID,
              "wsc_group_norm_nhwc (fp32): %d of %d channels at %d are not 16-byte groups", C, Ctot, coff);
    WSC_HIP(hipSetDevice(ctx->device));
    const size_t out_e = (size_t)N * Hd * Wd * Ctot;
    const size_t part_b = align_up(group_norm_partial_bytes(N, H, W, G), 256), stats_b = align_up(sizeof(float) * 2 * N * G, 256),
                 vec_b = align_up(sizeof(float) * C, 256);
    void *ws;
    WSC_TRY(wsc_ctx_workspace(ctx, act_bytes(out_e, prec) + part_b + stats_b + 2 * vec_b, &ws));
    char *p = (char *)ws;
    const Act yo = act_carve(p, out_e, prec);
    void *part = p, *stats = p + part_b;
    float *gamma = (float *)(p + part_b + stats_b), *beta = (float *)(p + part_b + stats_b + vec_b);
    WSC_TRY(wsc_ctx_upload_small(ctx, gamma, gamma_host, sizeof(float) * C));
    WSC_TRY(wsc_ctx_upload_small(ctx, beta, beta_host, sizeof(float) * C));
    WSC_TRY(launch_nchw_to_nhwc(ctx, y_dev, N * Hd * Wd, Ctot, 1, yo));
    WSC_TRY(launch_group_norm_stats(ctx, x_dev, N, H, W, C, G, eps, part, stats));
    WSC_TRY(launch_group_norm_apply(ctx, x_dev, stats, gamma, beta, N, H, W, C, G, up, relu, yo, Hd, Wd, Ctot, coff));
    return launch_act_to_f32(ctx, yo, out_e, y_dev);
}

int wsc_gap_linear_sigmoid(wsc_ctx *ctx, const float *feat_dev, int B, int hw, int F, const float *w_host, const float *bias_host, int C,
                           int sample_stride, int precision, float *score_dev) {
    WSC_CHECK(ctx && feat_dev && w_host && score_dev, WSC_ERR_INVALID, "wsc_gap_linear_sigmoid: null argument");
    wsc_precision prec;
    WSC_TRY(decode_precision(precision, &prec));
    WSC_CHECK(B > 0 && hw != 0 && hw > -(1 << 24) && hw < (1 << 24) && F > 0 && F <= 8192 && C > 0 && sample_stride >= 1 && sample_stride <= 2,
              WSC_ERR_INVALID, "wsc_gap_linear_sigmoid: B=%d, %d positions, F=%d, C=%d, sample stride %d", B, hw, F, C, sample_stride);
    WSC_HIP(hipSetDevice(ctx->device));
    const int npix = hw < 0 ? -hw : hw;
    const size_t in_e = (size_t)B * sample_stride * npix * F;
    const size_t w_b = align_up(sizeof(float) * (size_t)C * F, 256), b_b = align_up(sizeof(float) * C, 256);
    void *ws;
    WSC_TRY(wsc_ctx_workspace(ctx, act_bytes(in_e, prec) + w_b + b_b, &ws));
    char *p = (char *)ws;
    const Act feat = act_carve(p, in_e, prec);
    float *w = (float *)p, *bias = bias_host ? (float *)(p + w_b) : nullptr;
    WSC_TRY(wsc_ctx_upload_small(ctx, w, w_host, sizeof(float) * (size_t)C * F));
    if (bias) WSC_TRY(wsc_ctx_upload_small(ctx, bias, bias_host, sizeof(float) * C));
    WSC_TRY(launch_nchw_to_nhwc(ctx, feat_dev, B * sample_stride * npix, F, 1, feat));
    return launch_gap_linear_sigmoid(ctx, feat, B, hw, F, w, bias, C, score_dev, sample_stride);
}

int wsc_cam_flip_add(wsc_ctx *ctx, const float *head_dev, int B, int h, int w, int C, int Cs, float *cam_dev) {
    WSC_CHECK(ctx && head_dev && cam_dev, WSC_ERR_INVALID, "wsc_cam_flip_add: null argument");
    WSC_CHECK(B > 0 && h > 0 && w > 0 && C > 0 && C <= Cs, WSC_ERR_INVALID, "wsc_cam_flip_add: B=%d, %d x %d, %d of %d channels", B, h, w, C, Cs);
    WSC_HIP(hipSetDevice(ctx->device));
    return launch_flip_add(ctx, head_dev, B, h, w, C, Cs, cam_dev);
}

int wsc_irn_edge_finish(wsc_ctx *ctx, const float *e_dev, int He, int We, const float *d_dev, int Hd, int Wd, int B, int fh, int fw,
                        float ms0, float ms1, float *edge_dev, float *dp_dev) {
    WSC_CHECK(ctx && e_dev && d_dev && edge_dev && dp_dev, WSC_ERR_INVALID, "wsc_irn_edge_finish: null argument");
    WSC_CHECK(B > 0 && fh > 0 && fw > 0, WSC_ERR_INVALID, "wsc_irn_edge_finish: B=%d, feature size %d x %d", B, fh, fw);
    WSC_HIP(hipSetDevice(ctx->device));
    return launch_edge_finish(ctx, e_dev, He, We, d_dev, Hd, Wd, B, fh, fw, ms0, ms1, edge_dev, dp_dev);
}

}
```

wsss-analysis_amd/wsscam/_lib.py:

```python
import ctypes
import os
import re
import threading

import numpy as np

_HERE = os.path.dirname(os.path.abspath(__file__))
LIB_PATH = os.path.join(_HERE, "libwsscam.so")
HEADER_PATH = os.path.normpath(os.path.join(_HERE, "..", "..", "include", "wsscam.h"))

WSC_OK = 0
WSC_ERR_INVALID = -1
WSC_ERR_NO_DEVICE = -2
WSC_ERR_HIP = -3
WSC_ERR_MISSING_KEY = -4
WSC_ERR_SHAPE = -5
WSC_ERR_NOMEM = -6
WSC_ERR_KEY_RANGE = -7
WSC_ERR_CAPACITY = -8
WSC_ERR_RANGE = -9

ARCH_RESNET50_CAM = 0
ARCH_VGG16_CAM = 1
ARCH_M7_CAM = 2
ARCH_RESNET50_IRN = 3
ARCH_VGG16_IRN = 4
ARCH_M7_IRN = 5
ARCH_DEEPLAB_LFOV = 6
ARCH_DEEPLAB_ASPP = 7

PREC_BF16 = 0
PREC_BF16X3 = 1
PREC_F16 = 2
PREC_F16X3 = 3
PREC_F32 = 4
OPT_CRF_GAUSS_ON_CHIP, OPT_CRF_FUSED_BLUR, OPT_CRF_BLUR_ON_CHIP, OPT_CRF_RANK_BALLOT, OPT_CRF_EMBED_FULL, OPT_RW_TILED, \
    OPT_STEM_POOL_FUSED, OPT_CONV_WINDOW, OPT_CAM_HEAD_STREAM, OPT_CRF_MSG_IN_UPDATE = range(10)
OPT_DEFAULTS = {OPT_CRF_GAUSS_ON_CHIP: 1, OPT_CRF_FUSED_BLUR: 1, OPT_CRF_BLUR_ON_CHIP: 1, OPT_CRF_RANK_BALLOT: 0,
                OPT_CRF_EMBED_FULL: 0, OPT_RW_TILED: -1, OPT_STEM_POOL_FUSED: 1, OPT_CONV_WINDOW: 1, OPT_CAM_HEAD_STREAM: 1,
                OPT_CRF_MSG_IN_UPDATE: 1}
CONV_GENERIC = 0x100


class WscError(RuntimeError):
    def __init__(self, status, message):
        super().__init__("libwsscam error %d: %s" % (status, message))
        self.status = status


class TensorDesc(ctypes.Structure):
    _fields_ = [
        ("name", ctypes.c_char_p),
        ("data", ctypes.POINTER(ctypes.c_float)),
        ("ndim", ctypes.c_int32),
        ("shape", ctypes.c_int64 * 4),
    ]


class TraceOp(ctypes.Structure):
    _fields_ = [(n, ctypes.c_int32) for n in (
        "kind", "in_", "in2", "res", "Ho", "Wo", "C", "coff", "pitch", "kh", "kw", "stride", "pad", "dil", "relu", "affine2", "stride2",
        "pool_rule", "pool_k", "pool_stride", "pool_pad", "pool_avg", "fused_next")] + [("label", ctypes.c_char * 100)]


class TapeEntry(ctypes.Structure):
    _fields_ = [("name", ctypes.c_char * 32), ("Ho", ctypes.c_int32), ("Wo", ctypes.c_int32), ("C", ctypes.c_int32),
                ("offset", ctypes.c_int64)]


class GradEntry(ctypes.Structure):
    _fields_ = [("name", ctypes.c_char * 32), ("kh", ctypes.c_int32), ("kw", ctypes.c_int32), ("Cin", ctypes.c_int32),
                ("Cout", ctypes.c_int32), ("w_off", ctypes.c_int64), ("b_off", ctypes.c_int64)]


TRACE_CONV, TRACE_POOL, TRACE_GATHER, TRACE_HEAD = range(4)
TRACE_INPUT, TRACE_NONE = -1, -2

_lib = None

_vp = ctypes.c_void_p
_i = ctypes.c_int
_f = ctypes.c_float
_sz = ctypes.c_size_t
_d = ctypes.c_double

_SIGNATURES = {
    "wsc_version": (_i, []),
    "wsc_last_error": (ctypes.c_char_p, []),
    "wsc_ctx_create": (_i, [_i, _vp, ctypes.POINTER(_vp)]),
    "wsc_ctx_destroy": (None, [_vp]),
    "wsc_sync": (_i, [_vp]),
    "wsc_ctx_range_status": (_i, [_vp, ctypes.POINTER(_i), _i]),
    "wsc_ctx_wait": (_i, [_vp, _vp]),
    "wsc_ctx_mark": (_i, [_vp, _i]),
    "wsc_ctx_wait_mark": (_i, [_vp, _i]),
    "wsc_ctx_wait_for_mark": (_i, [_vp, _vp, _i]),
    "wsc_device_info": (_i, [_vp, ctypes.c_char_p, _sz, ctypes.POINTER(_i)]),
    "wsc_malloc": (_i, [_vp, _sz, ctypes.POINTER(_vp)]),
    "wsc_free": (_i, [_vp, _vp]),
    "wsc_memcpy_h2d": (_i, [_vp, _vp, _vp, _sz]),
    "wsc_memcpy_d2h": (_i, [_vp, _vp, _vp, _sz]),
    "wsc_memset": (_i, [_vp, _vp, _i, _sz]),
    "wsc_ctx_set_option": (_i, [_vp, _i, _i]),
    "wsc_host_alloc": (_i, [_vp, _sz, ctypes.POINTER(_vp)]),
    "wsc_host_free": (_i, [_vp, _vp]),
    "wsc_host_write_segments": (_i, [ctypes.c_char_p, _i, ctypes.POINTER(_vp), ctypes.POINTER(_sz)]),
    "wsc_memcpy_h2d_async": (_i, [_vp, _vp, _vp, _sz]),
    "wsc_memcpy_d2h_async": (_i, [_vp, _vp, _vp, _sz]),
    "wsc_profile_begin": (_i, [_vp]),
    "wsc_profile_end": (_i, [_vp, _i, _vp, _vp, _vp, ctypes.POINTER(_i)]),
    "wsc_profile_class_name": (ctypes.c_char_p, [_i]),
    "wsc_timer_begin": (_i, [_vp]),
    "wsc_timer_end": (_i, [_vp, ctypes.POINTER(_f)]),
    "wsc_net_create": (_i, [_vp, _i, ctypes.POINTER(TensorDesc), _i, _i, _i, ctypes.POINTER(_vp)]),
    "wsc_net_destroy": (None, [_vp]),
    "wsc_net_cam_size": (_i, [_vp, _i, ctypes.POINTER(_i)]),
    "wsc_net_feat_channels": (_i, [_vp, ctypes.POINTER(_i)]),
    "wsc_net_forward_cam": (_i, [_vp, _vp, _vp, _i, _i, _vp, _vp]),
    "wsc_net_forward_gradcam": (_i, [_vp, _vp, _vp, _i, _i, _i, _vp, _vp]),
    "wsc_net_forward_features": (_i, [_vp, _vp, _vp, _i, _i, _vp]),
    "wsc_net_cam_size_hw": (_i, [_vp, _i, _i, ctypes.POINTER(_i), ctypes.POINTER(_i)]),
    "wsc_net_forward_cam_hw": (_i, [_vp, _vp, _vp, _i, _i, _i, _vp, _vp]),
    "wsc_net_forward_edge": (_i, [_vp, _vp, _vp, _i, _i, _i, _i, _vp, _vp]),
    "wsc_rw_propagate": (_i, [_vp, _vp, _vp, _i, _i, _i, _vp, _vp, _vp, _i, _f, _i, _vp]),
    "wsc_rw_propagate_batch": (_i, [_vp, _i, _vp, _vp, _vp, _vp, _vp, _vp, _vp, _vp, _i, _f, _i, _vp]),
    "wsc_conv2d_nchw": (_i, [_vp, _vp, _i, _i, _i, _i, _vp, _i, _i, _i, _i, _i, _vp, _vp, _vp, _i, _i, _vp]),
    "wsc_conv2d_nchw_dil": (_i, [_vp, _vp, _i, _i, _i, _i, _vp, _i, _i, _i, _i, _i, _i, _vp, _vp, _vp, _i, _i, _vp]),
    "wsc_net_seg_size_hw": (_i, [_vp, _i, _i, ctypes.POINTER(_i), ctypes.POINTER(_i)]),
    "wsc_net_forward_seg": (_i, [_vp, _vp, _vp, _i, _i, _i, _f, _vp, _vp]),
    "wsc_net_seg_tape_plan": (_i, [_vp, _vp, _i, _i, _i, ctypes.POINTER(TapeEntry), _i, ctypes.POINTER(_i),
                                   ctypes.POINTER(ctypes.c_longlong)]),
    "wsc_net_forward_seg_tape": (_i, [_vp, _vp, _vp, _i, _i, _i, _f, _vp, ctypes.c_longlong, _vp, _vp]),
    "wsc_net_forward_seg_train": (_i, [_vp, _vp, _vp, _i, _i, _i, _f, _f, ctypes.c_ulonglong, ctypes.c_longlong, _vp, ctypes.c_longlong,
                                       _vp, _vp]),
    "wsc_seg_dropout_f32": (_i, [_vp, _vp, ctypes.c_longlong, ctypes.c_longlong, _f, ctypes.c_ulonglong, ctypes.c_longlong, _i, _vp, _vp]),
    "wsc_net_backward_seg_drop": (_i, [_vp, _vp, _i, _i, _i, _vp, ctypes.c_longlong, _vp, _vp, ctypes.c_longlong, _f]),
    "wsc_relu_bias_grad_scaled": (_i, [_vp, _vp, _vp, ctypes.c_longlong, _i, _f, _vp, _vp]),
    "wsc_seg_grad_create": (_i, [_vp, _vp, ctypes.POINTER(TensorDesc), _i, ctypes.POINTER(_vp)]),
    "wsc_seg_grad_destroy": (None, [_vp]),
    "wsc_seg_grad_layout": (_i, [_vp, ctypes.POINTER(GradEntry), _i, ctypes.POINTER(_i), ctypes.POINTER(ctypes.c_longlong)]),
    "wsc_net_backward_seg": (_i, [_vp, _vp, _i, _i, _i, _vp, ctypes.c_longlong, _vp, _vp, ctypes.c_longlong]),
    "wsc_conv2d_wgrad_nhwc": (_i, [_vp, _vp, _vp, _i, _i, _i, _i, _i, _i, _i, _i, _vp, _vp]),
    "wsc_seg_sgd_accumulate": (_i, [_vp, _vp, _vp, _vp, _vp, ctypes.c_longlong, _f, _i, _vp]),
    "wsc_seg_sgd_apply": (_i, [_vp, _vp, _vp, _vp, _vp, ctypes.c_longlong, _f, _f, _i]),
    "wsc_net_seg_load_params": (_i, [_vp, _vp, _vp, _vp, ctypes.c_longlong]),
    "wsc_conv2d_dgrad_nhwc": (_i, [_vp, _vp, _vp, _i, _i, _i, _i, _i, _i, _i, _vp]),
    "wsc_relu_bias_grad": (_i, [_vp, _vp, _vp, ctypes.c_longlong, _i, _vp, _vp]),
    "wsc_pool_same_grad_nhwc": (_i, [_vp, _vp, _vp, _i, _i, _i, _i, _i, _i, _vp]),
    "wsc_resize_bilinear_tf": (_i, [_vp, _vp, _i, _i, _i, _i, _vp, _i, _i]),
    "wsc_pool_same_nhwc": (_i, [_vp, _vp, _i, _i, _i, _i, _i, _i, _i, _vp]),
    "wsc_pool_tf_nhwc": (_i, [_vp, _vp, _i, _i, _i, _i, _i, _i, _i, _i, _vp]),
    "wsc_group_norm_nhwc": (_i, [_vp, _vp, _i, _i, _i, _i, _vp, _vp, _i, _f, _i, _i, _i, _i, _i, _i, _i, _vp]),
    "wsc_maxpool_nhwc": (_i, [_vp, _vp, _i, _i, _i, _i, _i, _i, _i, _i, _vp]),
    "wsc_gap_linear_sigmoid": (_i, [_vp, _vp, _i, _i, _i, _vp, _vp, _i, _i, _i, _vp]),
    "wsc_cam_flip_add": (_i, [_vp, _vp, _i, _i, _i, _i, _i, _vp]),
    "wsc_irn_edge_finish": (_i, [_vp, _vp, _i, _i, _vp, _i, _i, _i, _i, _i, _f, _f, _vp, _vp]),
    "wsc_fc8_softmax": (_i, [_vp, _vp, _i, ctypes.c_longlong, _i, _f, _vp, _vp]),
    "wsc_net_trace_plan": (_i, [_vp, _vp, _i, _i, _i, ctypes.POINTER(TraceOp), _i, ctypes.POINTER(_i)]),
    "wsc_net_forward_trace": (_i, [_vp, _vp, _vp, _i, _i, _i, ctypes.POINTER(ctypes.c_longlong), _i, _vp, ctypes.c_longlong]),
    "wsc_cam_postprocess": (_i, [_vp, _vp, _i, _i, _i, _i, _vp, _vp, _vp, _vp, _vp, _vp, _vp]),
    "wsc_cam_eval_confusion": (_i, [_vp, _vp, _i, _vp, _vp, _vp, _vp, _f, _vp, _i, _i, _vp, _vp]),
    "wsc_unary_from_maps": (_i, [_vp, _vp, _i, _i, _i, _f, _vp]),
    "wsc_cam_unary": (_i, [_vp, _vp, _i, _i, _i, _i, _i, _i, _f, _vp]),
    "wsc_cam_unary_pm": (_i, [_vp, _vp, _i, _i, _i, _i, _i, _i, _f, _vp]),
    "wsc_cam_sum_scales": (_i, [_vp, _vp, _i, _i, ctypes.c_longlong, _vp]),
    "wsc_cam_eval_confusion_nn": (_i, [_vp, _vp, _i, _vp, _vp, _vp, _vp, _vp, _vp, _i, _i, _vp, _vp]),
    "wsc_label_confusion_nn": (_i, [_vp, _vp, _i, _vp, _vp, _vp, _vp, _i, _i, _vp, _vp]),
    "wsc_sem_seg_finish": (_i, [_vp, _vp, _i, _vp, _vp, _vp, _vp, _vp, _vp, _i, _f, _vp]),
    "wsc_bilinear_resize": (_i, [_vp, _vp, _i, _i, _i, _vp, _i, _i]),
    "wsc_msf_input_u8": (_i, [_vp, _vp, _i, _vp, _vp, _i, _vp, _vp, _i, _i, _vp]),
    "wsc_resize_u8": (_i, [_vp, _vp, _i, _vp, _vp, _i, _i, _vp]),
    "wsc_label_unary_from_cam": (_i, [_vp, _vp, _i, _i, _i, _f, _f, _vp, _vp]),
    "wsc_ir_label_combine": (_i, [_vp, _vp, _vp, _vp, _i, _i, _i, _vp]),
    "wsc_dsrg_seed_grow": (_i, [_vp, _vp, _vp, _vp, _i, _i, _i, _i, _f, _f, _vp]),
    "wsc_seg_loss": (_i, [_vp, _i, _vp, _vp, _vp, _vp, _i, _i, _i, _i, _f, _vp, _f, _vp, _f, _vp, _vp, _vp]),
    "wsc_cue_maps": (_i, [_vp, _vp, _i, _i, _i, _i, _vp, _i, _vp, _i, _vp]),
    "wsc_cue_seeds": (_i, [_vp, _vp, _vp, _i, _i, _i, _i, _i, _d, _i, _d, _vp, _vp]),
    "wsc_seg_unary_nhwc": (_i, [_vp, _vp, _i, _i, _vp, _vp, _vp, _vp, _vp]),
    "wsc_seg_resize_argmax": (_i, [_vp, _vp, _i, _i, _vp, _vp, _vp, _vp, _vp]),
    "wsc_seg_preprocess_u8": (_i, [_vp, _vp, _i, _vp, _vp, _vp, _i, _i, _vp]),
    "wsc_seg_crf_image_u8": (_i, [_vp, _vp, _i, _i, _i, _vp, _i, _i, _vp]),
    "wsc_seg_crf_logprob": (_i, [_vp, _vp, _i, _i, ctypes.c_longlong, _f, _vp]),
    "wsc_seg_planes_from_nhwc": (_i, [_vp, _vp, _i, _i, ctypes.c_longlong, _vp]),
    "wsc_hsn_gradcam_post": (_i, [_vp, _vp, _i, _i, _i, _i, _i, _vp, _vp, _i, _i]),
    "wsc_hsn_voc_background": (_i, [_vp, _vp, _i, _i, _i, _vp, _i]),
    "wsc_hsn_class_mass": (_i, [_vp, _vp, _i, _i, _vp]),
    "wsc_hsn_background": (_i, [_vp, _vp, _i, _i, _i, _i, _i, _vp]),
    "wsc_cam_adp_modify": (_i, [_vp, _vp, _i, _i, _i, _i, _vp, _i, _vp, _i, _vp, _i, _vp, _i, _vp]),
    "wsc_hsn_cs_gradcam": (_i, [_vp, _vp, _i, _i, _i, _vp, _vp, _i, _i, _i, _vp, _i, _vp, _i, _vp, _vp, _vp]),
    "wsc_hsn_gather_unary": (_i, [_vp, _vp, _vp, _i, _i, _vp]),
    "wsc_crf_create": (_i, [_vp, _vp, _i, _i, _i, _f, _f, _f, ctypes.POINTER(_vp)]),
    "wsc_crf_destroy": (None, [_vp]),
    "wsc_crf_lattice_sizes": (_i, [_vp, _vp, _vp, _vp]),
    "wsc_crf_gaussian_on_chip": (_i, [_vp, _i]),
    "wsc_crf_inference": (_i, [_vp, _vp, _vp, _i, _f, _f, _i, _vp, _vp]),
    "wsc_crf_inference_pm": (_i, [_vp, _vp, _vp, _i, _f, _f, _i, _vp, _vp]),
    "wsc_crf_v_create": (_i, [_vp, _vp, _vp, _i, _f, _f, _f, ctypes.POINTER(_vp)]),
    "wsc_crf_v_destroy": (None, [_vp]),
    "wsc_crf_v_num_groups": (_i, [_vp]),
    "wsc_crf_v_inference": (_i, [_vp, _vp, _vp, _vp, _f, _f, _i, _vp, _vp]),
}


def header_symbols():
    with open(HEADER_PATH) as fh:
        text = fh.read()
    text = re.sub(r"/\*.*?\*/", "", text, flags=re.S)
    return sorted(set(re.findall(r"\b(wsc_[a-z0-9_]+)\s*\(", text)))


def load():
    global _lib
    if _lib is not None:
        return _lib
    if not os.path.exists(LIB_PATH):
        raise WscError(WSC_ERR_NO_DEVICE,
                       "libwsscam.so not built at %s -- run `python __graft_entry__.py` (there is no "
                       "CPU fallback for the product path)" % LIB_PATH)
    lib = ctypes.CDLL(LIB_PATH)
    for name, (res, args) in _SIGNATURES.items():
        fn = getattr(lib, name)
        fn.restype = res
        fn.argtypes = args
    _lib = lib
    return lib


def check_exports():
    lib = load()
    declared = header_symbols()
    missing = [s for s in declared if not hasattr(lib, s)]
    unbound = [s for s in declared if s not in _SIGNATURES]
    if missing or unbound:
        raise WscError(WSC_ERR_INVALID, "missing exports %s / unbound %s" % (missing, unbound))
    return declared


def check(status):
    if status != WSC_OK:
        raise WscError(status, load().wsc_last_error().decode("utf-8", "replace"))


def _ptr(x):
    if x is None:
        return None
    if isinstance(x, DeviceBuffer):
        return x.ptr
    if isinstance(x, np.ndarray):
        assert x.flags["C_CONTIGUOUS"]
        return x.ctypes.data
    if isinstance(x, int):
        return x
    if hasattr(x, "data_ptr"):
        return x.data_ptr()
    raise TypeError("cannot take a pointer of %r" % type(x))


class StackChain:

    SLOT = 7

    def __init__(self):
        self._lock = threading.Lock()
        self._last = None

    def run(self, ctx, enqueue):
        with self._lock:
            prev = self._last
            if prev is not None and prev is not ctx:
                ctx.wait_for_mark(prev, self.SLOT)
            try:
                return enqueue()
            finally:
                ctx.mark(self.SLOT)
                self._last = ctx


class Context:

    def __init__(self, device=0, stream=None):
# ... 328 lines not shown


class SegGrad:

    def __init__(self, net, state_dict):
        self.ctx = net.ctx
        self.net = net
        descs, keep = make_tensor_descs(state_dict)
        h = _vp()
        check(self.ctx._lib.wsc_seg_grad_create(self.ctx.h, net.h, descs, len(descs), ctypes.byref(h)))
        del keep
        self.h = h
        n, elems = _i(), ctypes.c_longlong()
        check(self.ctx._lib.wsc_seg_grad_layout(h, None, 0, ctypes.byref(n), ctypes.byref(elems)))
        ent = (GradEntry * n.value)()
        check(self.ctx._lib.wsc_seg_grad_layout(h, ent, n.value, ctypes.byref(n), ctypes.byref(elems)))
        self.layout = {e.name.decode(): {"k": e.kh, "Cin": e.Cin, "Cout": e.Cout, "w_off": e.w_off, "b_off": e.b_off} for e in ent}
        self.grad_elems = elems.value

    def close(self):
        if getattr(self, "h", None) and self.ctx.h:
            self.ctx._lib.wsc_seg_grad_destroy(self.h)
        self.h = None

    def __del__(self):
        try:
            self.close()
        except Exception:
            pass

    def backward(self, B, H, W, tape_dev, tape_elems, dfc8_dev, grad_dev, grad_elems=None):
        check(self.ctx._lib.wsc_net_backward_seg(self.ctx.h, self.h, int(B), int(H), int(W), _ptr(tape_dev), int(tape_elems), _ptr(dfc8_dev),
                                                 _ptr(grad_dev), int(self.grad_elems if grad_elems is None else grad_elems)))

    def backward_drop(self, B, H, W, tape_dev, tape_elems, dfc8_dev, grad_dev, drop_prob, grad_elems=None):
        check(self.ctx._lib.wsc_net_backward_seg_drop(self.ctx.h, self.h, int(B), int(H), int(W), _ptr(tape_dev), int(tape_elems),
                                                      _ptr(dfc8_dev), _ptr(grad_dev),
                                                      int(self.grad_elems if grad_elems is None else grad_elems), float(drop_prob)))

    def sgd_accumulate(self, param_dev, grad_dev, accum_dev, weight_decay, accum_num, l2_dev=None, elems=None, ctx=None):
        run = ctx or self.ctx
        check(self.ctx._lib.wsc_seg_sgd_accumulate(run.h, self.h, _ptr(param_dev), _ptr(grad_dev), _ptr(accum_dev),
                                                   int(self.grad_elems if elems is None else elems), float(weight_decay), int(accum_num),
                                                   _ptr(l2_dev)))

    def sgd_apply(self, param_dev, accum_dev, mom_dev, lr, momentum, clear_accum=True, elems=None, ctx=None):
        run = ctx or self.ctx
        check(self.ctx._lib.wsc_seg_sgd_apply(run.h, self.h, _ptr(param_dev), _ptr(accum_dev), _ptr(mom_dev),
                                              int(self.grad_elems if elems is None else elems), float(lr), float(momentum), int(bool(clear_accum))))

    def load_params(self, param_dev, elems=None, net=None, ctx=None):
        run = ctx or self.ctx
        check(self.ctx._lib.wsc_net_seg_load_params(run.h, (net or self.net).h, self.h, _ptr(param_dev),
                                                    int(self.grad_elems if elems is None else elems)))


def conv2d_wgrad_nhwc(ctx, x_dev, dy_dev, N, H, W, Cin, Cout, k, dil, splits, dw_dev, db_dev):
    check(ctx._lib.wsc_conv2d_wgrad_nhwc(ctx.h, _ptr(x_dev), _ptr(dy_dev), int(N), int(H), int(W), int(Cin), int(Cout), int(k), int(dil),
                                         int(splits), _ptr(dw_dev), _ptr(db_dev)))


def conv2d_dgrad_nhwc(ctx, dy_dev, w, N, H, W, Cin, Cout, k, dil, dx_dev):
    w = np.ascontiguousarray(w, dtype=np.float32)
    assert w.shape == (k, k, Cin, Cout)
    check(ctx._lib.wsc_conv2d_dgrad_nhwc(ctx.h, _ptr(dy_dev), _ptr(w), int(N), int(H), int(W), int(Cin), int(Cout), int(k), int(dil),
                                         _ptr(dx_dev)))


def relu_bias_grad(ctx, y_dev, dy_dev, M, C, dz_dev, db_dev):
    check(ctx._lib.wsc_relu_bias_grad(ctx.h, _ptr(y_dev), _ptr(dy_dev), int(M), int(C), _ptr(dz_dev), _ptr(db_dev)))


def relu_bias_grad_scaled(ctx, y_dev, dy_dev, M, C, scale, dz_dev, db_dev):
    check(ctx._lib.wsc_relu_bias_grad_scaled(ctx.h, _ptr(y_dev), _ptr(dy_dev), int(M), int(C), float(scale), _ptr(dz_dev), _ptr(db_dev)))


def seg_dropout_f32(ctx, x_dev, elems, first, drop_prob, seed, step, site, y_dev, keep_dev=None):
    check(ctx._lib.wsc_seg_dropout_f32(ctx.h, _ptr(x_dev), int(elems), int(first), float(drop_prob), int(seed) & 0xFFFFFFFFFFFFFFFF, int(step),
                                       int(site), _ptr(y_dev), _ptr(keep_dev)))


def pool_same_grad_nhwc(ctx, x_dev, dy_dev, N, H, W, C, avg, stride, dx_dev):
    check(ctx._lib.wsc_pool_same_grad_nhwc(ctx.h, _ptr(x_dev), _ptr(dy_dev), int(N), int(H), int(W), int(C), int(bool(avg)), int(stride),
                                           _ptr(dx_dev)))


def _key_table(keys_per_image, B=None):
    per = [np.asarray(k, dtype=np.int32).reshape(-1) for k in list(keys_per_image)[:B]]
    key_off = np.zeros(len(per) + 1, dtype=np.int32)
    key_off[1:] = np.cumsum([len(k) for k in per])
    return np.concatenate(per + [np.zeros(0 if key_off[-1] else 1, np.int32)]), key_off


def _size_table(sizes, B):
    return np.ascontiguousarray(sizes, dtype=np.int32).reshape(B, 2)


def cam_postprocess(ctx, cam_dev, B, C, h, w, sizes, keys_per_image, strided_dev=None, highres_dev=None):
    size_hw = _size_table(sizes, B)
    keys, key_off = _key_table(keys_per_image, B)
    s_off = np.zeros(B, dtype=np.int64)
    h_off = np.zeros(B, dtype=np.int64)
    shapes = []
    s_tot = 0
    h_tot = 0
    for b in range(B):
        H0, W0 = int(size_hw[b, 0]), int(size_hw[b, 1])
        h4, w4 = (H0 - 1) // 4 + 1, (W0 - 1) // 4 + 1
        K = int(key_off[b + 1] - key_off[b])
        s_off[b] = s_tot
        h_off[b] = h_tot
        s_tot += K * h4 * w4
        h_tot += K * H0 * W0
        shapes.append((K, h4, w4, H0, W0))
    if strided_dev is None:
        strided_dev = ctx.alloc(max(s_tot, 1) * 4)
    if highres_dev is None:
        highres_dev = ctx.alloc(max(h_tot, 1) * 4)
    check(ctx._lib.wsc_cam_postprocess(ctx.h, _ptr(cam_dev), B, C, h, w, size_hw.ctypes.data, keys.ctypes.data,
                                       key_off.ctypes.data, s_off.ctypes.data, h_off.ctypes.data,
                                       _ptr(strided_dev), _ptr(highres_dev)))
    return strided_dev, highres_dev, s_off, h_off, shapes


def conv2d_nchw(ctx, x_dev, N, Cin, H, W, w, stride, pad, scale=None, shift=None, residual_dev=None, relu=False,
                precision=PREC_BF16, y_dev=None, dil=1):
    w = np.ascontiguousarray(w, dtype=np.float32)
    Cout, _, kh, kw = w.shape
    dil = int(dil)
    Ho, Wo = (H + 2 * pad - ((kh - 1) * dil + 1)) // stride + 1, (W + 2 * pad - ((kw - 1) * dil + 1)) // stride + 1
    if y_dev is None:
        y_dev = ctx.alloc(N * Cout * Ho * Wo * 4)
    sc = None if scale is None else np.ascontiguousarray(scale, dtype=np.float32)
    sh = None if shift is None else np.ascontiguousarray(shift, dtype=np.float32)
    if dil == 1:
        check(ctx._lib.wsc_conv2d_nchw(ctx.h, _ptr(x_dev), N, Cin, H, W, w.ctypes.data, Cout, kh, kw, stride, pad,
                                       None if sc is None else sc.ctypes.data, None if sh is None else sh.ctypes.data,
                                       _ptr(residual_dev), int(relu), precision, _ptr(y_dev)))
    else:
        conv2d_nchw_dil(ctx, x_dev, N, Cin, H, W, w, stride, pad, dil, sc, sh, residual_dev, relu, precision, y_dev)
    return y_dev, (N, Cout, Ho, Wo)


def conv2d_nchw_dil(ctx, x_dev, N, Cin, H, W, w, stride, pad, dil, scale, shift, residual_dev, relu, precision, y_dev):
    w = np.ascontiguousarray(w, dtype=np.float32)
    Cout, _, kh, kw = w.shape
    sc = None if scale is None else np.ascontiguousarray(scale, dtype=np.float32)
    sh = None if shift is None else np.ascontiguousarray(shift, dtype=np.float32)
    check(ctx._lib.wsc_conv2d_nchw_dil(ctx.h, _ptr(x_dev), N, Cin, H, W, w.ctypes.data, Cout, kh, kw, stride, pad, int(dil),
                                       None if sc is None else sc.ctypes.data, None if sh is None else sh.ctypes.data,
                                       _ptr(residual_dev), int(relu), precision, _ptr(y_dev)))


def resize_bilinear_tf(ctx, src_dev, B, h, w, C, H, W, dst_dev=None):
    if dst_dev is None:
        dst_dev = ctx.alloc(B * H * W * C * 4)
    check(ctx._lib.wsc_resize_bilinear_tf(ctx.h, _ptr(src_dev), int(B), int(h), int(w), int(C), _ptr(dst_dev), int(H), int(W)))
    return dst_dev


def pool_same_nhwc(ctx, x_dev, N, H, W, C, avg, stride, precision, y_dev=None):
    Ho, Wo = -(-H // stride), -(-W // stride)
    if y_dev is None:
        y_dev = ctx.alloc(N * Ho * Wo * C * 4)
    check(ctx._lib.wsc_pool_same_nhwc(ctx.h, _ptr(x_dev), int(N), int(H), int(W), int(C), int(bool(avg)), int(stride), int(precision),
                                      _ptr(y_dev)))
    return y_dev, (N, Ho, Wo, C)


def pool_tf_nhwc(ctx, x_dev, N, H, W, C, k, stride, same, precision, y_dev=None):
    from .net.common import pooled_size

    row = (int(k), int(stride), "same" if same else "valid")
    try:
        Ho, Wo = pooled_size(H, [row]), pooled_size(W, [row])
    except ValueError:
        Ho = Wo = 0
    if y_dev is None:
        y_dev = ctx.alloc(max(N * Ho * Wo * C, 1) * 4)
    check(ctx._lib.wsc_pool_tf_nhwc(ctx.h, _ptr(x_dev), int(N), int(H), int(W), int(C), int(k), int(stride), int(same),
                                    int(precision), _ptr(y_dev)))
    return y_dev, (N, Ho, Wo, C)


def group_norm_nhwc(ctx, x_dev, N, H, W, C, gamma, beta, G, eps, up, relu, Hd, Wd, Ctot, coff, precision, y_dev):
    g = None if gamma is None else np.ascontiguousarray(gamma, dtype=np.float32)
    b = None if beta is None else np.ascontiguousarray(beta, dtype=np.float32)
    check(ctx._lib.wsc_group_norm_nhwc(ctx.h, _ptr(x_dev), int(N), int(H), int(W), int(C), _ptr(g), _ptr(b), int(G), float(eps), int(up),
                                       int(bool(relu)), int(Hd), int(Wd), int(Ctot), int(coff), int(precision), _ptr(y_dev)))
    return y_dev, (N, Hd, Wd, Ctot)


def maxpool_nhwc(ctx, x_dev, N, H, W, C, k, stride, pad, precision, y_dev=None):
    Ho, Wo = (H + 2 * pad - k) // stride + 1, (W + 2 * pad - k) // stride + 1
    if y_dev is None:
        y_dev = ctx.alloc(max(N * Ho * Wo * C, 1) * 4)
    check(ctx._lib.wsc_maxpool_nhwc(ctx.h, _ptr(x_dev), int(N), int(H), int(W), int(C), int(k), int(stride), int(pad), int(precision),
                                    _ptr(y_dev)))
    return y_dev, (N, Ho, Wo, C)


def gap_linear_sigmoid(ctx, feat_dev, B, hw, F, w, bias, sample_stride, precision, score_dev=None):
    w = np.ascontiguousarray(w, dtype=np.float32)
    C = w.shape[0]
    b = None if bias is None else np.ascontiguousarray(bias, dtype=np.float32)
    if score_dev is None:
        score_dev = ctx.alloc(max(B * C, 1) * 4)
    check(ctx._lib.wsc_gap_linear_sigmoid(ctx.h, _ptr(feat_dev), int(B), int(hw), int(F), _ptr(w), _ptr(b), int(C), int(sample_stride),
                                          int(precision), _ptr(score_dev)))
    return score_dev, (B, C)


def cam_flip_add(ctx, head_dev, B, h, w, C, Cs, cam_dev=None):
    if cam_dev is None:
        cam_dev = ctx.alloc(max(B * C * h * w, 1) * 4)
    check(ctx._lib.wsc_cam_flip_add(ctx.h, _ptr(head_dev), int(B), int(h), int(w), int(C), int(Cs), _ptr(cam_dev)))
    return cam_dev, (B, C, h, w)


def irn_edge_finish(ctx, e_dev, He, We, d_dev, Hd, Wd, B, fh, fw, ms0, ms1, edge_dev=None, dp_dev=None):
    n = max(B * fh * fw, 1)
    if edge_dev is None:
        edge_dev = ctx.alloc(n * 4)
    if dp_dev is None:
        dp_dev = ctx.alloc(2 * n * 4)
    check(ctx._lib.wsc_irn_edge_finish(ctx.h, _ptr(e_dev), int(He), int(We), _ptr(d_dev), int(Hd), int(Wd), int(B), int(fh), int(fw),
                                       float(ms0), float(ms1), _ptr(edge_dev), _ptr(dp_dev)))
    return edge_dev, dp_dev


def fc8_softmax(ctx, fc8_devs, M, C, prob_dev, min_prob=1e-4, sum_dev=None):
    ptrs = (_vp * len(fc8_devs))(*[_ptr(d) for d in fc8_devs])
    check(ctx._lib.wsc_fc8_softmax(ctx.h, ptrs, len(fc8_devs), int(M), int(C), float(min_prob), _ptr(sum_dev), _ptr(prob_dev)))


def cam_eval_confusion(ctx, highres_dev, sizes, keys_per_image, highres_off, bg_thres, gt_dev, n_class, confusion_dev,
                       pred_dev=None, ignore_label=255):
    B = len(sizes)
    size_hw = _size_table(sizes, B)
    keys, key_off = _key_table(keys_per_image, B)
    h_off = np.ascontiguousarray(highres_off, dtype=np.int64)
    check(ctx._lib.wsc_cam_eval_confusion(ctx.h, _ptr(highres_dev), B, size_hw.ctypes.data, keys.ctypes.data,
                                          key_off.ctypes.data, h_off.ctypes.data, float(bg_thres), _ptr(gt_dev),
                                          int(n_class), int(ignore_label), _ptr(pred_dev), _ptr(confusion_dev)))


def cam_eval_confusion_nn(ctx, maps_dev, src_sizes, out_sizes, keys_per_image, maps_off, gt_dev, n_class, confusion_dev,
                          pred_dev=None, ignore_label=255):
    B = len(src_sizes)
    src_hw = _size_table(src_sizes, B)
    out_hw = _size_table(out_sizes, B)
    keys, key_off = _key_table(keys_per_image, B)
    m_off = np.ascontiguousarray(maps_off, dtype=np.int64)
    check(ctx._lib.wsc_cam_eval_confusion_nn(ctx.h, _ptr(maps_dev), B, src_hw.ctypes.data, out_hw.ctypes.data, keys.ctypes.data,
                                             key_off.ctypes.data, m_off.ctypes.data, _ptr(gt_dev), int(n_class),
                                             int(ignore_label), _ptr(pred_dev), _ptr(confusion_dev)))


def label_confusion_nn(ctx, labels_dev, src_sizes, out_sizes, labels_off, gt_dev, n_class, confusion_dev, pred_dev=None,
                       ignore_label=255):
    B = len(src_sizes)
    src_hw = _size_table(src_sizes, B)
    out_hw = _size_table(out_sizes, B)
    off = np.ascontiguousarray(labels_off, dtype=np.int64)
    check(ctx._lib.wsc_label_confusion_nn(ctx.h, _ptr(labels_dev), B, src_hw.ctypes.data, out_hw.ctypes.data, off.ctypes.data,
                                          _ptr(gt_dev), int(n_class), int(ignore_label), _ptr(pred_dev), _ptr(confusion_dev)))


def sem_seg_finish(ctx, rw_dev, rw_off, khw, up_hw, out_hw, keys_per_image, has_bg, bg_thres, label_dev):
    B = len(khw)
    keys, key_off = _key_table(keys_per_image, B)
    off = np.ascontiguousarray(rw_off, dtype=np.int64)
    a, u, o = (np.ascontiguousarray(v, dtype=np.int32).reshape(B, -1) for v in (khw, up_hw, out_hw))
    check(ctx._lib.wsc_sem_seg_finish(ctx.h, _ptr(rw_dev), B, off.ctypes.data, a.ctypes.data, u.ctypes.data, o.ctypes.data,
                                      keys.ctypes.data, key_off.ctypes.data, int(bool(has_bg)), float(bg_thres), _ptr(label_dev)))


def unary_from_maps(ctx, maps_dev, B, C, N, bg_value, unary_dev):
    check(ctx._lib.wsc_unary_from_maps(ctx.h, _ptr(maps_dev), B, C, N, float(bg_value), _ptr(unary_dev)))


def cam_unary(ctx, cam_dev, B, C, h, w, H0, W0, bg_value, unary_dev, pixel_major=False):
    fn = ctx._lib.wsc_cam_unary_pm if pixel_major else ctx._lib.wsc_cam_unary
    check(fn(ctx.h, _ptr(cam_dev), B, C, h, w, H0, W0, float(bg_value), _ptr(unary_dev)))


def cam_sum_scales(ctx, cam_dev, n_images, n_scales, map_elems, out_dev):
    check(ctx._lib.wsc_cam_sum_scales(ctx.h, _ptr(cam_dev), int(n_images), int(n_scales), int(map_elems), _ptr(out_dev)))


def bilinear_resize(ctx, src_dev, C, h, w, dst_dev, H, W):
    check(ctx._lib.wsc_bilinear_resize(ctx.h, _ptr(src_dev), C, h, w, _ptr(dst_dev), H, W))


class Crf:

    def __init__(self, ctx, rgb_dev, B, H, W, g_sxy, bi_sxy, bi_srgb):
        self.ctx = ctx
        self.B, self.H, self.W = B, H, W
        h = _vp()
        check(ctx._lib.wsc_crf_create(ctx.h, _ptr(rgb_dev), B, H, W, float(g_sxy), float(bi_sxy), float(bi_srgb),
                                      ctypes.byref(h)))
        self.h = h

    def close(self):
        if getattr(self, "h", None) and self.ctx.h:
# ... 248 lines not shown
```

Measured before the change: 2646 images/s.

## Fuse bottleneck conv3 1x1 with next block's conv1 1x1 into one kernel

Adds a fused HIP kernel that computes a 64->256 1x1 conv with BN, residual add and ReLU, then feeds the resulting trunk tile from LDS straight into the following 256->64 1x1 conv. The network forward detects such conv pairs and launches the fused kernel, enabled by default through a new option. The aim is to avoid re-reading the 256-channel trunk activation from global memory and to save one launch per pair. In exchange the kernel uses large LDS (80KB) and extra barriers, which may lower occupancy.

Result: no change. 2657 images/s (median of 2 runs) (+0.4%).

```diff
diff --git a/__graft_entry__.py b/__graft_entry__.py
--- a/__graft_entry__.py
+++ b/__graft_entry__.py
@@ -9,7 +9,7 @@
 ORACLE_DIR = os.path.join(ROOT, "oracle")
 ORACLE_OUT = os.path.join(ORACLE_DIR, "_build", "libdensecrf_ref.so")
 
-HIP_SOURCES = ["api.hip", "conv_igemm.hip", "misc_kernels.hip", "net.hip", "cam_tail.hip", "crf.hip", "irn_kernels.hip", "rw.hip", "hsn.hip", "input.hip", "ir_label.hip", "stem_pool.hip", "cam_head.hip", "conv_f32.hip", "dsrg.hip", "cue_seeds.hip", "seg_eval.hip", "deeplab.hip", "seg_chain.hip", "seg_loss.hip", "pool.hip", "seg_grad.hip", "seg_sgd.hip", "seg_dropout.hip"]
+HIP_SOURCES = ["api.hip", "conv_igemm.hip", "misc_kernels.hip", "net.hip", "cam_tail.hip", "crf.hip", "irn_kernels.hip", "rw.hip", "hsn.hip", "input.hip", "ir_label.hip", "stem_pool.hip", "cam_head.hip", "conv_f32.hip", "dsrg.hip", "cue_seeds.hip", "seg_eval.hip", "deeplab.hip", "seg_chain.hip", "seg_loss.hip", "pool.hip", "seg_grad.hip", "seg_sgd.hip", "seg_dropout.hip", "conv_pair.hip"]
 EXTRA_FLAGS = {"crf.hip": ["-ffp-contract=off"], "input.hip": ["-ffp-contract=off"], "deeplab.hip": ["-ffp-contract=off"],
                "seg_chain.hip": ["-ffp-contract=off"],
                "seg_sgd.hip": ["-ffp-contract=off"],
diff --git a/include/wsscam.h b/include/wsscam.h
--- a/include/wsscam.h
+++ b/include/wsscam.h
@@ -55,7 +55,8 @@
     WSC_OPT_CONV_WINDOW = 7,
     WSC_OPT_CAM_HEAD_STREAM = 8,
     WSC_OPT_CRF_MSG_IN_UPDATE = 9,
-    WSC_OPT_COUNT = 10
+    WSC_OPT_CONV_PAIR = 10,
+    WSC_OPT_COUNT = 11
 } wsc_option;
 
 typedef struct wsc_crf wsc_crf;
@@ -141,6 +142,10 @@
                         int Cout, int kh, int kw, int stride, int pad, int dil, const float *scale_host,
                         const float *shift_host, const float *residual_dev, int relu, int precision,
                         float *y_dev);
+
+int wsc_conv_pair_nchw(wsc_ctx *ctx, const float *x_dev, int N, int H, int W, const float *w3_host, const float *scale3_host,
+                       const float *shift3_host, const float *residual_dev, const float *w1_host, const float *scale1_host,
+                       const float *shift1_host, float *trunk_dev, float *y_dev);
 
 
 int wsc_net_seg_size_hw(const wsc_net *net, int H, int W, int *h_out, int *w_out);
diff --git a/profiles/conv_pair_one.py b/profiles/conv_pair_one.py
--- /dev/null
+++ b/profiles/conv_pair_one.py
@@ -0,0 +1,46 @@
+import os
+import sys
+
+import numpy as np
+
+ROOT = os.path.dirname(os.path.dirname(os.path.abspath(__file__)))
+sys.path.insert(0, os.path.join(ROOT, "wsss-analysis_amd"))
+from wsscam import _lib
+
+
+def main():
+    a = [int(v) for v in sys.argv[1:]]
+    N, H, W, reps = (a + [64, 81, 81, 20][len(a):])[:4]
+    rng = np.random.default_rng(0)
+    ctx = _lib.Context(0)
+    x = ctx.to_device(np.maximum(rng.normal(0, 1, (N, 64, H, W)), 0).astype(np.float32))
+    res = ctx.to_device(np.maximum(rng.normal(0, 1, (N, 256, H, W)), 0).astype(np.float32))
+    w3 = (rng.normal(0, 1, (256, 64, 1, 1)) * np.sqrt(2.0 / 64)).astype(np.float32)
+    w1 = (rng.normal(0, 1, (64, 256, 1, 1)) * np.sqrt(2.0 / 256)).astype(np.float32)
+    s3, b3 = np.ones(256, np.float32), np.zeros(256, np.float32)
+    s1, b1 = np.ones(64, np.float32), np.zeros(64, np.float32)
+    t, y = ctx.alloc(N * 256 * H * W * 4), ctx.alloc(N * 64 * H * W * 4)
+    M = N * H * W
+    print("pair at %d x %d x %d (M = %d), %d launches each" % (N, H, W, M, reps))
+    tot = {}
+    for rnd in range(2):
+        for pair in (0, 1):
+            ctx.set_option(_lib.OPT_CONV_PAIR, pair)
+            _lib.conv_pair_nchw(ctx, x, N, H, W, w3, s3, b3, res, w1, s1, b1, t, y)
+            ctx.sync()
+            ctx.profile_begin()
+            for _ in range(reps):
+                _lib.conv_pair_nchw(ctx, x, N, H, W, w3, s3, b3, res, w1, s1, b1, t, y)
+            prof = ctx.profile_end()
+            us = 0.0
+            for name, (calls, ms, work) in sorted(prof.items()):
+                if name.startswith("conv_igemm"):
+                    us += ms / reps * 1e3
+                    print("  pair=%d  %-40s %d launches, %.1f us per call" % (pair, name, calls // reps, ms / reps * 1e3))
+            tot.setdefault(pair, []).append(us)
+            print("pair=%d round %d: %.1f us" % (pair, rnd, us))
+    print("two launches %s us, one kernel %s us" % (["%.1f" % v for v in tot[0]], ["%.1f" % v for v in tot[1]]))
+
+
+if __name__ == "__main__":
+    main()
diff --git a/wsss-analysis_amd/csrc/common.h b/wsss-analysis_amd/csrc/common.h
--- a/wsss-analysis_amd/csrc/common.h
+++ b/wsss-analysis_amd/csrc/common.h
@@ -139,7 +139,7 @@
     };
     PinSlot pin_ring[PIN_SLOTS];
     int pin_next = 0;
-    int opt[WSC_OPT_COUNT] = {1, 1, 1, 0, 0, -1, 1, 1, 1, 1};
+    int opt[WSC_OPT_COUNT] = {1, 1, 1, 0, 0, -1, 1, 1, 1, 1, 1};
     void *zero_page = nullptr;
     unsigned *range_host = nullptr, *range_dev = nullptr;
     hipEvent_t ev0 = nullptr, ev1 = nullptr;
@@ -335,6 +335,11 @@
     }
 };
 int conv_igemm_launch(wsc_ctx *ctx, const ConvLaunch &p);
+__device__ __forceinline__ int lds_off(int row, int slot) {
+    return row * 128 + ((slot ^ ((row >> 1) & 7)) << 4);
+}
+bool conv_pair_fits(const ConvLaunch &a, const ConvLaunch &b);
+int conv_pair_launch(wsc_ctx *ctx, const ConvLaunch &a, const ConvLaunch &b);
 int conv_f32_launch(wsc_ctx *ctx, const ConvLaunch &p);
 int launch_cam_head(wsc_ctx *ctx, Act x, int M, int K, const bf16_t *w, int Kw, int CoutPad, const float *s1, const float *b1,
                     int C, int relu, float *y);
diff --git a/wsss-analysis_amd/csrc/conv_igemm.hip b/wsss-analysis_amd/csrc/conv_igemm.hip
--- a/wsss-analysis_amd/csrc/conv_igemm.hip
+++ b/wsss-analysis_amd/csrc/conv_igemm.hip
@@ -36,10 +36,6 @@
     int spare2, spare3;
     unsigned *range;
 };
-
-__device__ __forceinline__ int lds_off(int row, int slot) {
-    return row * 128 + ((slot ^ ((row >> 1) & 7)) << 4);
-}
 
 __device__ __forceinline__ void decode_row(const ConvKArgs &p, int m, int &n, int &ho, int &wo) {
     const unsigned t1 = __umulhi(p.div_howo_mul, (unsigned)m);
diff --git a/wsss-analysis_amd/csrc/conv_pair.hip b/wsss-analysis_amd/csrc/conv_pair.hip
--- /dev/null
+++ b/wsss-analysis_amd/csrc/conv_pair.hip
@@ -0,0 +1,372 @@
+#include "common.h"
+
+#include <type_traits>
+
+namespace {
+
+constexpr int CP_MID = 64;
+constexpr int CP_TRUNK = 256;
+constexpr int CP_BM = 64;
+constexpr int CP_REGION_A = 65536, CP_REGION_B = 16384;
+constexpr int CP_LDS = CP_REGION_A + CP_REGION_B;
+constexpr int CP_TILE = 8192;
+
+struct ConvPairArgs {
+    const bf16_t *x;
+    long long x_lo_delta;
+    const bf16_t *w3;
+    const float *s3, *b3;
+    const bf16_t *res, *res_lo;
+    bf16_t *t, *t_lo;
+    const bf16_t *w1;
+    const float *s1, *b1;
+    bf16_t *y, *y_lo;
+    int M, nblocks, Kw3, Kw1;
+    unsigned *range;
+};
+
+typedef unsigned u32x4_t __attribute__((ext_vector_type(4)));
+
+__device__ __forceinline__ int ct_off(int row, int col) { return row * 64 + ((((col >> 2) ^ row) & 15) << 2) + (col & 3); }
+
+__device__ __forceinline__ f32x16_t mfma16(const u32x4_t &a, const u32x4_t &b, const f32x16_t &c) {
+    return __builtin_amdgcn_mfma_f32_32x32x16_f16(__builtin_bit_cast(f16x8_t, a), __builtin_bit_cast(f16x8_t, b), c, 0, 0, 0);
+}
+
+template <bool RES>
+__device__ __forceinline__ void epilogue8(const f32x4_t &q0, const f32x4_t &q1, const float (&s)[8], const float (&b)[8], const uint4 &rh,
+                                          const uint4 &rl, uint32_t (&hw)[4], uint32_t (&lw)[4]) {
+    float v[8];
+#pragma unroll
+    for (int j = 0; j < 4; ++j) {
+        v[j] = q0[j] * s[j] + b[j];
+        v[4 + j] = q1[j] * s[4 + j] + b[4 + j];
+    }
+    if (RES) {
+        const uint32_t rw[4] = {rh.x, rh.y, rh.z, rh.w};
+#pragma unroll
+        for (int j = 0; j < 4; ++j) {
+            v[2 * j] += f16_to_f32((bf16_t)(rw[j] & 0xffffu));
+            v[2 * j + 1] += f16_to_f32((bf16_t)(rw[j] >> 16));
+        }
+        const uint32_t lr[4] = {rl.x, rl.y, rl.z, rl.w};
+#pragma unroll
+        for (int j = 0; j < 4; ++j) {
+            v[2 * j] += f16_to_f32((bf16_t)(lr[j] & 0xffffu));
+            v[2 * j + 1] += f16_to_f32((bf16_t)(lr[j] >> 16));
+        }
+    }
+#pragma unroll
+    for (int j = 0; j < 4; ++j) {
+        const float c0 = __builtin_amdgcn_fmed3f(v[2 * j], 0.f, 65504.f), c1 = __builtin_amdgcn_fmed3f(v[2 * j + 1], 0.f, 65504.f);
+        const _Float16 h0 = (_Float16)c0;
+        const _Float16 h1 = (_Float16)c1;
+        hw[j] = (uint32_t)__builtin_bit_cast(uint16_t, h0) | ((uint32_t)__builtin_bit_cast(uint16_t, h1) << 16);
+        const _Float16 l0 = (_Float16)(c0 - (float)h0), l1 = (_Float16)(c1 - (float)h1);
+        lw[j] = (uint32_t)__builtin_bit_cast(uint16_t, l0) | ((uint32_t)__builtin_bit_cast(uint16_t, l1) << 16);
+    }
+}
+
+__global__ __launch_bounds__(256, 2) void conv_pair_kernel(ConvPairArgs p) {
+    __shared__ __attribute__((aligned(16))) char smem[CP_LDS];
+    char *const regA = smem, *const regB = smem + CP_REGION_A;
+
+    const int t = threadIdx.x;
+    const int lane = t & 63;
+    const int wv = __builtin_amdgcn_readfirstlane(t >> 6);
+    const int l31 = lane & 31, kgrp = lane >> 5;
+
+    int tile;
+    {
+        const int bid = blockIdx.x;
+        const int xcd = bid & 7;
+        const int q = p.nblocks >> 3, r = p.nblocks & 7;
+        tile = (xcd < r ? xcd * (q + 1) : r * (q + 1) + (xcd - r) * q) + (bid >> 3);
+    }
+    const int m0 = tile * CP_BM;
+
+    const int c8 = t & 7, r0 = t >> 3;
+    int mrow[2];
+#pragma unroll
+    for (int ps = 0; ps < 2; ++ps) mrow[ps] = m0 + ps * 32 + r0;
+
+    uint4 rres[4][2], rres_lo[4][2];
+    auto fetch_res = [&]() {
+#pragma unroll
+        for (int q = 0; q < 4; ++q)
+#pragma unroll
+            for (int ps = 0; ps < 2; ++ps) {
+                const int mc = mrow[ps] < p.M ? mrow[ps] : p.M - 1;
+                const unsigned o = (unsigned)mc * (unsigned)CP_TRUNK + (unsigned)(q * 64 + c8 * 8);
+                rres[q][ps] = *reinterpret_cast<const uint4 *>(p.res + o);
+                rres_lo[q][ps] = *reinterpret_cast<const uint4 *>(p.res_lo + o);
+            }
+    };
+    const int srow = lane >> 3, slot = lane & 7;
+    auto dma = [&](const bf16_t *g, char *dst) {
+        __builtin_amdgcn_global_load_lds((const __attribute__((address_space(1))) void *)g, (__attribute__((address_space(3))) void *)dst, 16, 0, 0);
+    };
+#pragma unroll
+    for (int i = 0; i < 4; ++i) {
+        const int idx = wv * 4 + i, kt = idx >> 3, r = (idx & 7) * 8 + srow;
+        const int m = m0 + r < p.M ? m0 + r : p.M - 1;
+        const int ks = slot ^ ((r >> 1) & 7);
+        dma(p.x + ((long long)m * CP_MID + kt * 32 + (ks & 3) * 8 + ((ks & 4) ? p.x_lo_delta : 0ll)), regB + idx * 1024);
+    }
+#pragma unroll
+    for (int i = 0; i < 16; ++i) {
+        const int idx = wv * 16 + i, kt = idx >> 5, r = (idx & 31) * 8 + srow;
+        const int ks = slot ^ ((r >> 1) & 7);
+        dma(p.w3 + (r * p.Kw3 + kt * 64 + ks * 8), regA + idx * 1024);
+    }
+    const bf16_t *w1src[2];
+#pragma unroll
+    for (int i = 0; i < 2; ++i) {
+        const int r = (wv * 2 + i) * 8 + srow;
+        w1src[i] = p.w1 + (r * p.Kw1 + (slot ^ ((r >> 1) & 7)) * 8);
+    }
+    auto issue_w1 = [&](int kt, int at) {
+#pragma unroll
+        for (int i = 0; i < 2; ++i) dma(w1src[i] + kt * 64, smem + at + (wv * 2 + i) * 1024);
+    };
+
+    const unsigned lds0 = (unsigned)(uintptr_t)(__attribute__((address_space(3))) char *)smem;
+    float *const ct = reinterpret_cast<float *>(regB);
+
+    __syncthreads();
+
+    f32x16_t acc[2][2];
+#pragma unroll
+    for (int mi = 0; mi < 2; ++mi)
+#pragma unroll
+        for (int ni = 0; ni < 2; ++ni)
+#pragma unroll
+            for (int r = 0; r < 16; ++r) acc[mi][ni][r] = 0.f;
+    {
+        unsigned offA[4], offB[4];
+#pragma unroll
+        for (int pr = 0; pr < 4; ++pr) {
+            offA[pr] = lds0 + CP_REGION_A + lds_off(l31, pr * 2 + kgrp);
+            offB[pr] = lds0 + lds_off(wv * 64 + l31, pr * 2 + kgrp);
+        }
+#pragma unroll
+        for (int kt = 0; kt < 2; ++kt) {
+            if (kt == 1) fetch_res();
+#pragma unroll
+            for (int sl = 0; sl < 2; ++sl) {
+                u32x4_t fah[2], fal[2], fbh[2], fbl[2];
+#pragma unroll
+                for (int mi = 0; mi < 2; ++mi) {
+                    asm volatile("ds_read_b128 %0, %1 offset:%2" : "=v"(fah[mi]) : "v"(offA[sl]), "n"(kt * CP_TILE + mi * 4096) : "memory");
+                    asm volatile("ds_read_b128 %0, %1 offset:%2" : "=v"(fal[mi]) : "v"(offA[2 + sl]), "n"(kt * CP_TILE + mi * 4096) : "memory");
+                }
+#pragma unroll
+                for (int ni = 0; ni < 2; ++ni) {
+                    asm volatile("ds_read_b128 %0, %1 offset:%2" : "=v"(fbh[ni]) : "v"(offB[sl]), "n"(kt * 32768 + ni * 4096) : "memory");
+                    asm volatile("ds_read_b128 %0, %1 offset:%2" : "=v"(fbl[ni]) : "v"(offB[2 + sl]), "n"(kt * 32768 + ni * 4096) : "memory");
+                }
+                asm volatile("s_waitcnt lgkmcnt(0)" ::: "memory");
+                __builtin_amdgcn_sched_barrier(0);
+#pragma unroll
+                for (int mi = 0; mi < 2; ++mi)
+#pragma unroll
+                    for (int ni = 0; ni < 2; ++ni) acc[mi][ni] = mfma16(fal[mi], fbh[ni], acc[mi][ni]);
+#pragma unroll
+                for (int mi = 0; mi < 2; ++mi)
+#pragma unroll
+                    for (int ni = 0; ni < 2; ++ni) acc[mi][ni] = mfma16(fah[mi], fbl[ni], acc[mi][ni]);
+#pragma unroll
+                for (int mi = 0; mi < 2; ++mi)
+#pragma unroll
+                    for (int ni = 0; ni < 2; ++ni) acc[mi][ni] = mfma16(fah[mi], fbh[ni], acc[mi][ni]);
+            }
+        }
+    }
+    __syncthreads();
+
+    unsigned ovf = 0u;
+#pragma unroll
+    for (int q = 0; q < 4; ++q) {
+        const int c = q * 64 + c8 * 8;
+        float s[8], b[8];
+        {
+            const f32x4_t sa = *reinterpret_cast<const f32x4_t *>(p.s3 + c), sb = *reinterpret_cast<const f32x4_t *>(p.s3 + c + 4);
+            const f32x4_t ba = *reinterpret_cast<const f32x4_t *>(p.b3 + c), bb = *reinterpret_cast<const f32x4_t *>(p.b3 + c + 4);
+#pragma unroll
+            for (int j = 0; j < 4; ++j) {
+                s[j] = sa[j];
+                s[4 + j] = sb[j];
+                b[j] = ba[j];
+                b[4 + j] = bb[j];
+            }
+        }
+        if (wv == q) {
+#pragma unroll
+            for (int mi = 0; mi < 2; ++mi)
+#pragma unroll
+                for (int ni = 0; ni < 2; ++ni)
+#pragma unroll
+                    for (int r = 0; r < 16; ++r)
+                        ct[ct_off(mi * 32 + (r & 3) + 8 * (r >> 2) + 4 * kgrp, ni * 32 + l31)] = acc[mi][ni][r];
+        }
+        __syncthreads();
+        f32x4_t q0[2], q1[2];
+#pragma unroll
+        for (int ps = 0; ps < 2; ++ps) {
+            q0[ps] = *reinterpret_cast<const f32x4_t *>(ct + ct_off(ps * 32 + r0, c8 * 8));
+            q1[ps] = *reinterpret_cast<const f32x4_t *>(ct + ct_off(ps * 32 + r0, c8 * 8 + 4));
+        }
+        __syncthreads();
+        if (q == 3) {
+            issue_w1(0, CP_REGION_A);
+            issue_w1(1, CP_REGION_A + CP_TILE);
+        }
+#pragma unroll
+        for (int ps = 0; ps < 2; ++ps) {
+            uint32_t hw[4], lw[4];
+            epilogue8<true>(q0[ps], q1[ps], s, b, rres[q][ps], rres_lo[q][ps], hw, lw);
+            const uint4 vh = make_uint4(hw[0], hw[1], hw[2], hw[3]), vl = make_uint4(lw[0], lw[1], lw[2], lw[3]);
+            if (mrow[ps] < p.M) {
+                ovf |= half2_at_ceiling(hw[0]) | half2_at_ceiling(hw[1]) | half2_at_ceiling(hw[2]) | half2_at_ceiling(hw[3]);
+                const unsigned o = (unsigned)mrow[ps] * (unsigned)CP_TRUNK + (unsigned)c;
+                *reinterpret_cast<uint4 *>(p.t + o) = vh;
+                *reinterpret_cast<uint4 *>(p.t_lo + o) = vl;
+            }
+            char *const at = regA + (q * 2 + (c8 >> 2)) * CP_TILE;
+            *reinterpret_cast<uint4 *>(at + lds_off(ps * 32 + r0, c8 & 3)) = vh;
+            *reinterpret_cast<uint4 *>(at + lds_off(ps * 32 + r0, 4 + (c8 & 3))) = vl;
+        }
+    }
+    if (ovf & 0x80008000u) *p.range = (unsigned)CP_TRUNK;
+
+    const int wm = wv >> 1, wn = wv & 1;
+    f32x16_t acc2;
+#pragma unroll
+    for (int r = 0; r < 16; ++r) acc2[r] = 0.f;
+    {
+        unsigned offA[4], offBa[4], offBb[4];
+#pragma unroll
+        for (int pr = 0; pr < 4; ++pr) {
+            offA[pr] = lds0 + lds_off(wm * 32 + l31, pr * 2 + kgrp);
+            offBa[pr] = lds0 + lds_off(wn * 32 + l31, pr * 2 + kgrp);
+            offBb[pr] = offBa[pr] + CP_REGION_A;
+        }
+        auto step = [&](auto kt_c) __attribute__((always_inline)) {
+            constexpr int kt = decltype(kt_c)::value;
+            constexpr int b_at = kt < 2 ? kt * CP_TILE : (kt == 2 ? 0 : (kt - 3) * CP_TILE);
+            const unsigned(&offB)[4] = kt <= 2 ? offBb : offBa;
+            if (kt < 2 || kt == 7) asm volatile("s_waitcnt vmcnt(0) lgkmcnt(0)" ::: "memory");
+            else asm volatile("s_waitcnt vmcnt(2)" ::: "memory");
+            __builtin_amdgcn_s_barrier();
+            __builtin_amdgcn_sched_barrier(0);
+            if (kt == 1) issue_w1(2, CP_REGION_A);
+            if (kt >= 1 && kt + 2 < 8) issue_w1(kt + 2, (kt - 1) * CP_TILE);
+            __builtin_amdgcn_sched_barrier(0);
+#pragma unroll
+            for (int sl = 0; sl < 2; ++sl) {
+                u32x4_t fah, fal, fbh, fbl;
+                asm volatile("ds_read_b128 %0, %1 offset:%2" : "=v"(fah) : "v"(offA[sl]), "n"(kt * CP_TILE) : "memory");
+                asm volatile("ds_read_b128 %0, %1 offset:%2" : "=v"(fal) : "v"(offA[2 + sl]), "n"(kt * CP_TILE) : "memory");
+                asm volatile("ds_read_b128 %0, %1 offset:%2" : "=v"(fbh) : "v"(offB[sl]), "n"(b_at) : "memory");
+                asm volatile("ds_read_b128 %0, %1 offset:%2" : "=v"(fbl) : "v"(offB[2 + sl]), "n"(b_at) : "memory");
+                asm volatile("s_waitcnt lgkmcnt(0)" ::: "memory");
+                __builtin_amdgcn_sched_barrier(0);
+                acc2 = mfma16(fal, fbh, acc2);
+                acc2 = mfma16(fah, fbl, acc2);
+                acc2 = mfma16(fah, fbh, acc2);
+            }
+        };
+        step(std::integral_constant<int, 0>{});
+        step(std::integral_constant<int, 1>{});
+        step(std::integral_constant<int, 2>{});
+        step(std::integral_constant<int, 3>{});
+        step(std::integral_constant<int, 4>{});
+        step(std::integral_constant<int, 5>{});
+        step(std::integral_constant<int, 6>{});
+        step(std::integral_constant<int, 7>{});
+    }
+    __syncthreads();
+
+#pragma unroll
+    for (int r = 0; r < 16; ++r) ct[ct_off(wm * 32 + (r & 3) + 8 * (r >> 2) + 4 * kgrp, wn * 32 + l31)] = acc2[r];
+    float s[8], b[8];
+    {
+        const int c = c8 * 8;
+        const f32x4_t sa = *reinterpret_cast<const f32x4_t *>(p.s1 + c), sb = *reinterpret_cast<const f32x4_t *>(p.s1 + c + 4);
+        const f32x4_t ba = *reinterpret_cast<const f32x4_t *>(p.b1 + c), bb = *reinterpret_cast<const f32x4_t *>(p.b1 + c + 4);
+#pragma unroll
+        for (int j = 0; j < 4; ++j) {
+            s[j] = sa[j];
+            s[4 + j] = sb[j];
+            b[j] = ba[j];
+            b[4 + j] = bb[j];
+        }
+    }
+    __syncthreads();
+    unsigned ovf2 = 0u;
+#pragma unroll
+    for (int ps = 0; ps < 2; ++ps) {
+        const f32x4_t q0 = *reinterpret_cast<const f32x4_t *>(ct + ct_off(ps * 32 + r0, c8 * 8));
+        const f32x4_t q1 = *reinterpret_cast<const f32x4_t *>(ct + ct_off(ps * 32 + r0, c8 * 8 + 4));
+        uint32_t hw[4], lw[4];
+        const uint4 none = make_uint4(0, 0, 0, 0);
+        epilogue8<false>(q0, q1, s, b, none, none, hw, lw);
+        if (mrow[ps] < p.M) {
+            ovf2 |= half2_at_ceiling(hw[0]) | half2_at_ceiling(hw[1]) | half2_at_ceiling(hw[2]) | half2_at_ceiling(hw[3]);
+            const unsigned o = (unsigned)mrow[ps] * (unsigned)CP_MID + (unsigned)(c8 * 8);
+            *reinterpret_cast<uint4 *>(p.y + o) = make_uint4(hw[0], hw[1], hw[2], hw[3]);
+            *reinterpret_cast<uint4 *>(p.y_lo + o) = make_uint4(lw[0], lw[1], lw[2], lw[3]);
+        }
+    }
+    if (ovf2 & 0x80008000u) *p.range = (unsigned)CP_MID;
+}
+
+bool pointwise_relu(const ConvLaunch &l, int Cin, int Cout) {
+    return l.prec == WSC_PREC_F16X3 && l.form == CONV_FORM_GENERIC && l.kh == 1 && l.kw == 1 && l.stride == 1 && l.pad == 0 && l.relu &&
+           l.Cin == Cin && l.Cout == Cout && l.CoutPad == Cout && !l.generic && !l.x2 && l.s2 == nullptr && l.y_f32 == nullptr &&
+           (l.ldy == 0 || l.ldy == Cout) && l.Ho == l.H && l.Wo == l.W && l.operands_match() && l.x.hi && l.x.lo && l.y.hi && l.y.lo;
+}
+
+}
+
+bool conv_pair_fits(const ConvLaunch &a, const ConvLaunch &b) {
+    if (!pointwise_relu(a, CP_MID, CP_TRUNK) || !pointwise_relu(b, CP_TRUNK, CP_MID)) return false;
+    if (!a.res.hi || !a.res.lo || b.res) return false;
+    if (b.x.hi != a.y.hi || b.x.lo != a.y.lo || a.N != b.N || a.H != b.H || a.W != b.W) return false;
+    const long long M = (long long)a.N * a.Ho * a.Wo;
+    if (M < 1 || M * CP_TRUNK >= (1ll << 31)) return false;
+    const size_t ybytes = (size_t)M * CP_MID * sizeof(bf16_t), tbytes = (size_t)M * CP_TRUNK * sizeof(bf16_t);
+    auto overlap = [](const void *p, size_t pn, const void *q, size_t qn) {
+        return (const char *)p < (const char *)q + qn && (const char *)q < (const char *)p + pn;
+    };
+    for (const void *y : {b.y.hi, b.y.lo}) {
+        for (const void *o : {a.res.hi, a.res.lo, a.y.hi, a.y.lo})
+            if (overlap(y, ybytes, o, tbytes)) return false;
+        for (const void *o : {a.x.hi, a.x.lo})
+            if (overlap(y, ybytes, o, ybytes)) return false;
+    }
+    return true;
+}
+
+int conv_pair_launch(wsc_ctx *ctx, const ConvLaunch &a, const ConvLaunch &b) {
+    WSC_CHECK(conv_pair_fits(a, b), WSC_ERR_INVALID, "conv pair: not a 64 -> 256 (+ residual) / 256 -> 64 pair of pointwise f16x3 layers");
+    const ConvKLayout k3 = conv_k_layout(1, 1, CP_MID, CONV_FORM_GENERIC, a.prec), k1 = conv_k_layout(1, 1, CP_TRUNK, CONV_FORM_GENERIC, b.prec);
+    WSC_CHECK(k3.interleaved && k1.interleaved && k3.nk == 2 && k1.nk == 8 && k3.kstep == 64 && k1.kstep == 64, WSC_ERR_INVALID,
+              "conv pair: the packed-K layout is not [32 hi | 32 lo] K-steps");
+    ConvPairArgs p = {};
+    p.x = a.x.h16();
+    p.x_lo_delta = (long long)(a.x.h16_lo() - a.x.h16());
+    p.w3 = (const bf16_t *)a.w; p.s3 = a.s1; p.b3 = a.b1;
+    p.res = a.res.h16(); p.res_lo = a.res.h16_lo();
+    p.t = a.y.h16(); p.t_lo = a.y.h16_lo();
+    p.w1 = (const bf16_t *)b.w; p.s1 = b.s1; p.b1 = b.b1;
+    p.y = b.y.h16(); p.y_lo = b.y.h16_lo();
+    p.M = a.N * a.Ho * a.Wo;
+    p.nblocks = (p.M + CP_BM - 1) / CP_BM;
+    p.Kw3 = k3.Kw; p.Kw1 = k1.Kw;
+    p.range = ctx->range_dev;
+    WscKernelTimer timer(ctx, WSC_K_CONV128, 2.0 * p.M * (double)CP_MID * CP_TRUNK * 2.0);
+    hipLaunchKernelGGL(conv_pair_kernel, dim3(p.nblocks), dim3(256), 0, ctx->stream, p);
+    WSC_HIP(hipGetLastError());
+    return WSC_OK;
+}
diff --git a/wsss-analysis_amd/csrc/net.hip b/wsss-analysis_amd/csrc/net.hip
--- a/wsss-analysis_amd/csrc/net.hip
+++ b/wsss-analysis_amd/csrc/net.hip
@@ -271,6 +271,7 @@
     add_pool_op(net, POOL_TORCH, 3, 2, 1, false, 0, 1);
     net->taps.push_back((int)net->ops.size() - 1);
     int cur = 1;
+    int idle = -1;
     const int blocks[4] = {3, 4, 6, 3};
     const int strides[4] = {1, 2, 2, 1};
     for (int L = 0; L < 4; ++L) {
@@ -278,8 +279,10 @@
             const std::string pre = "resnet50.layer" + std::to_string(L + 1) + "." + std::to_string(bi);
             const int s = bi == 0 ? strides[L] : 1;
             int f[3], nf = 0;
+            if (idle >= 0 && idle != cur) f[nf++] = idle;
             for (int i = 0; i < 4 && nf < 3; ++i)
-                if (i != cur) f[nf++] = i;
+                if (i != cur && i != idle) f[nf++] = i;
+            idle = f[2];
             WSC_TRY(resnet_conv(net, d, pre + ".conv1", pre + ".bn1", 1, 0, 1, CONV_FORM_GENERIC, cur, f[0], -1));
             bool fuse_here = false;
             if (net->prec != WSC_PREC_F32 && has(d, pre + ".downsample.0.weight") && has(d, pre + ".conv3.weight")) {
@@ -786,29 +789,43 @@
         WSC_TRY(launch_nhwc3_to_nhwc4(ctx, x_dev, N, S, SW, xin));
     } else if (in_pad > 0) WSC_TRY(launch_nchw_to_nhwc4_pad(ctx, x_dev, N, S, SW, in_h, in_w, in_pad, xin));
     else WSC_TRY(launch_nchw_to_nhwc4(ctx, x_dev, N, S, SW, xin));
+    auto conv_op_launch = [&](size_t i) {
+        const Op &op = net->ops[i];
+        const OpDims &d = pl.ops[i];
+        const ConvW &c = net->convs[op.conv];
+        ConvLaunch L = conv_launch(c, net->prec);
+        L.x = op.in < 0 ? xin : buf[op.in];
+        if (op.res >= 0) L.res = buf[op.res];
+        L.y = buf[op.out].at(op.coff);
+        L.ldy = op.pitch;
+        if (op.in2 >= 0) {
+            L.x2 = buf[op.in2];
+            L.H2 = d.H2; L.W2 = d.W2; L.C2 = d.C2; L.stride2 = op.ps;
+        }
+        L.N = N; L.H = d.H; L.W = d.W; L.Ho = d.Ho; L.Wo = d.Wo;
+        if (c.form == CONV_FORM_STEM_ROWS && op.in < 0) on_padded_input(L, in_h, in_w);
+        return L;
+    };
+    bool paired = false;
     for (size_t i = 0; i < net->ops.size(); ++i) {
         const Op &op = net->ops[i];
         const OpDims &d = pl.ops[i];
         const Act src = op.in < 0 ? xin : buf[op.in];
         if (fused_stem && i == 0) continue;
-        if (fused_stem && i == 1) {
+        if (paired) {
+            paired = false;
+        } else if (fused_stem && i == 1) {
             const ConvW &c0 = net->convs[net->ops[0].conv];
             WSC_TRY(launch_stem_pool(ctx, xin, N, S, SW, (const bf16_t *)c0.w, conv_k_layout(c0.kh, c0.kw, c0.Cin, c0.form, net->prec).Kw, c0.s1,
                                      c0.b1, c0.relu, buf[op.out]));
         } else if (op.type == OP_CONV) {
-            const ConvW &c = net->convs[op.conv];
-            ConvLaunch L = conv_launch(c, net->prec);
-            L.x = src;
-            if (op.res >= 0) L.res = buf[op.res];
-            L.y = buf[op.out].at(op.coff);
-            L.ldy = op.pitch;
-            if (op.in2 >= 0) {
-                L.x2 = buf[op.in2];
-                L.H2 = d.H2; L.W2 = d.W2; L.C2 = d.C2; L.stride2 = op.ps;
+            const ConvLaunch L = conv_op_launch(i);
+            if (ctx->opt[WSC_OPT_CONV_PAIR] != 0 && i + 1 < net->ops.size() && net->ops[i + 1].type == OP_CONV && net->ops[i + 1].in == op.out) {
+                const ConvLaunch L2 = conv_op_launch(i + 1);
+                paired = conv_pair_fits(L, L2);
+                if (paired) WSC_TRY(conv_pair_launch(ctx, L, L2));
             }
-            L.N = N; L.H = d.H; L.W = d.W; L.Ho = d.Ho; L.Wo = d.Wo;
-            if (c.form == CONV_FORM_STEM_ROWS && op.in < 0) on_padded_input(L, in_h, in_w);
-            WSC_TRY(conv_igemm_launch(ctx, L));
+            if (!paired) WSC_TRY(conv_igemm_launch(ctx, L));
         } else if (op.type == OP_GATHER) {
             WSC_TRY(launch_gather_strided(ctx, src, N, d.H, d.W, d.C, op.ps, d.Ho, d.Wo, buf[op.out].at(op.coff), op.pitch));
         } else {
@@ -1750,6 +1767,57 @@
     return st;
 }
 
+int wsc_conv_pair_nchw(wsc_ctx *ctx, const float *x_dev, int N, int H, int W, const float *w3_host, const float *scale3_host,
+                       const float *shift3_host, const float *residual_dev, const float *w1_host, const float *scale1_host,
+                       const float *shift1_host, float *trunk_dev, float *y_dev) {
+    WSC_CHECK(ctx && x_dev && w3_host && scale3_host && shift3_host && residual_dev && w1_host && scale1_host && shift1_host && trunk_dev &&
+                  y_dev, WSC_ERR_INVALID, "wsc_conv_pair_nchw: null argument");
+    WSC_CHECK(N > 0 && H > 0 && W > 0 && (long long)N * H * W * 256 < (1ll << 31), WSC_ERR_INVALID, "wsc_conv_pair_nchw: N=%d, %d x %d", N, H, W);
+    WSC_HIP(hipSetDevice(ctx->device));
+    const int Cmid = 64, Ct = 256;
+    const wsc_precision prec = WSC_PREC_F16X3;
+    wsc_net tmp;
+    tmp.ctx = ctx;
+    tmp.prec = prec;
+    auto cleanup = [&]() {
+        (void)hipStreamSynchronize(ctx->stream);
+        for (void *p : tmp.allocs) (void)hipFree(p);
+    };
+    HostTensor t3, t1;
+    t3.data = w3_host; t3.ndim = 4; t3.shape[0] = Ct; t3.shape[1] = Cmid; t3.shape[2] = 1; t3.shape[3] = 1;
+    t1.data = w1_host; t1.ndim = 4; t1.shape[0] = Cmid; t1.shape[1] = Ct; t1.shape[2] = 1; t1.shape[3] = 1;
+    ConvW c3, c1;
+    int st = make_conv(&tmp, &t3, 1, 0, 1, CONV_FORM_GENERIC, std::vector<float>(scale3_host, scale3_host + Ct),
+                       std::vector<float>(shift3_host, shift3_host + Ct), nullptr, nullptr, &c3);
+    if (st == WSC_OK)
+        st = make_conv(&tmp, &t1, 1, 0, 1, CONV_FORM_GENERIC, std::vector<float>(scale1_host, scale1_host + Cmid),
+                       std::vector<float>(shift1_host, shift1_host + Cmid), nullptr, nullptr, &c1);
+    const size_t M = (size_t)N * H * W;
+    void *ws = nullptr;
+    if (st == WSC_OK) st = wsc_ctx_workspace(ctx, 2 * act_bytes(M * Cmid, prec) + 2 * act_bytes(M * Ct, prec), &ws);
+    if (st != WSC_OK) { cleanup(); return st; }
+    char *p = (char *)ws;
+    const Act xi = act_carve(p, M * Cmid, prec), ri = act_carve(p, M * Ct, prec), ti = act_carve(p, M * Ct, prec), yo = act_carve(p, M * Cmid, prec);
+    st = launch_nchw_to_nhwc(ctx, x_dev, N, Cmid, H * W, xi);
+    if (st == WSC_OK) st = launch_nchw_to_nhwc(ctx, residual_dev, N, Ct, H * W, ri);
+    if (st == WSC_OK) {
+        ConvLaunch a = conv_launch(c3, prec), b = conv_launch(c1, prec);
+        a.x = xi; a.res = ri; a.y = ti;
+        b.x = ti; b.y = yo;
+        a.N = b.N = N; a.H = b.H = a.Ho = b.Ho = H; a.W = b.W = a.Wo = b.Wo = W;
+        if (ctx->opt[WSC_OPT_CONV_PAIR] != 0) {
+            st = conv_pair_launch(ctx, a, b);
+        } else {
+            st = conv_igemm_launch(ctx, a);
+            if (st == WSC_OK) st = conv_igemm_launch(ctx, b);
+        }
+    }
+    if (st == WSC_OK) st = launch_nhwc_to_nchw(ctx, ti, N, Ct, H * W, trunk_dev);
+    if (st == WSC_OK) st = launch_nhwc_to_nchw(ctx, yo, N, Cmid, H * W, y_dev);
+    cleanup();
+    return st;
+}
+
 int wsc_group_norm_nhwc(wsc_ctx *ctx, const float *x_dev, int N, int H, int W, int C, const float *gamma_host, const float *beta_host,
                         int G, float eps, int up, int relu, int Hd, int Wd, int Ctot, int coff, int precision, float *y_dev) {
     WSC_CHECK(ctx && x_dev && gamma_host && beta_host && y_dev, WSC_ERR_INVALID, "wsc_group_norm_nhwc: null argument");
diff --git a/wsss-analysis_amd/wsscam/_lib.py b/wsss-analysis_amd/wsscam/_lib.py
--- a/wsss-analysis_amd/wsscam/_lib.py
+++ b/wsss-analysis_amd/wsscam/_lib.py
@@ -35,10 +35,10 @@
 PREC_F16X3 = 3
 PREC_F32 = 4
 OPT_CRF_GAUSS_ON_CHIP, OPT_CRF_FUSED_BLUR, OPT_CRF_BLUR_ON_CHIP, OPT_CRF_RANK_BALLOT, OPT_CRF_EMBED_FULL, OPT_RW_TILED, \
-    OPT_STEM_POOL_FUSED, OPT_CONV_WINDOW, OPT_CAM_HEAD_STREAM, OPT_CRF_MSG_IN_UPDATE = range(10)
+    OPT_STEM_POOL_FUSED, OPT_CONV_WINDOW, OPT_CAM_HEAD_STREAM, OPT_CRF_MSG_IN_UPDATE, OPT_CONV_PAIR = range(11)
 OPT_DEFAULTS = {OPT_CRF_GAUSS_ON_CHIP: 1, OPT_CRF_FUSED_BLUR: 1, OPT_CRF_BLUR_ON_CHIP: 1, OPT_CRF_RANK_BALLOT: 0,
                 OPT_CRF_EMBED_FULL: 0, OPT_RW_TILED: -1, OPT_STEM_POOL_FUSED: 1, OPT_CONV_WINDOW: 1, OPT_CAM_HEAD_STREAM: 1,
-                OPT_CRF_MSG_IN_UPDATE: 1}
+                OPT_CRF_MSG_IN_UPDATE: 1, OPT_CONV_PAIR: 1}
 CONV_GENERIC = 0x100
 
 
@@ -126,6 +126,7 @@
     "wsc_rw_propagate_batch": (_i, [_vp, _i, _vp, _vp, _vp, _vp, _vp, _vp, _vp, _vp, _i, _f, _i, _vp]),
     "wsc_conv2d_nchw": (_i, [_vp, _vp, _i, _i, _i, _i, _vp, _i, _i, _i, _i, _i, _vp, _vp, _vp, _i, _i, _vp]),
     "wsc_conv2d_nchw_dil": (_i, [_vp, _vp, _i, _i, _i, _i, _vp, _i, _i, _i, _i, _i, _i, _vp, _vp, _vp, _i, _i, _vp]),
+    "wsc_conv_pair_nchw": (_i, [_vp, _vp, _i, _i, _i, _vp, _vp, _vp, _vp, _vp, _vp, _vp, _vp, _vp]),
     "wsc_net_seg_size_hw": (_i, [_vp, _i, _i, ctypes.POINTER(_i), ctypes.POINTER(_i)]),
     "wsc_net_forward_seg": (_i, [_vp, _vp, _vp, _i, _i, _i, _f, _vp, _vp]),
     "wsc_net_seg_tape_plan": (_i, [_vp, _vp, _i, _i, _i, ctypes.POINTER(TapeEntry), _i, ctypes.POINTER(_i),
@@ -760,6 +761,18 @@
                                        _ptr(residual_dev), int(relu), precision, _ptr(y_dev)))
 
 
+def conv_pair_nchw(ctx, x_dev, N, H, W, w3, scale3, shift3, residual_dev, w1, scale1, shift1, trunk_dev=None, y_dev=None):
+    a = [np.ascontiguousarray(v, dtype=np.float32) for v in (w3, scale3, shift3, w1, scale1, shift1)]
+    assert a[0].shape[:2] == (256, 64) and a[3].shape[:2] == (64, 256) and a[1].size == a[2].size == 256 and a[4].size == a[5].size == 64
+    if trunk_dev is None:
+        trunk_dev = ctx.alloc(N * 256 * H * W * 4)
+    if y_dev is None:
+        y_dev = ctx.alloc(N * 64 * H * W * 4)
+    check(ctx._lib.wsc_conv_pair_nchw(ctx.h, _ptr(x_dev), N, H, W, a[0].ctypes.data, a[1].ctypes.data, a[2].ctypes.data, _ptr(residual_dev),
+                                      a[3].ctypes.data, a[4].ctypes.data, a[5].ctypes.data, _ptr(trunk_dev), _ptr(y_dev)))
+    return trunk_dev, y_dev
+
+
 def resize_bilinear_tf(ctx, src_dev, B, h, w, C, H, W, dst_dev=None):
     if dst_dev is None:
         dst_dev = ctx.alloc(B * H * W * C * 4)
```
